# NVIDIA-RTX/RTXPT

Measured on AMD Instinct MI355X. Metric: Mrays/s at 4K 4spp 8-bounce bistro-like (extend + shadow rays / wall time of pt_render), higher is better.
Workload: dtype f32; 1 GPU; C3 bistro-like street canyon, 2808008 triangles, 64 materials, 32 textures 1024^2, 7368 emissive-triangle + env-quad lights, 3840x2160, 4 spp, 8 bounces, NEE 5 candidates + RR, lp types binary16 (reference default), environment cube 2048 BC6H (reference default on D3D12); BVH builder=PLOC + parallel re-insertion + cost-driven wide nodes, built on device, buildMs 79.1 (host part 0.0), 275780 wide n; parallelism=pixel-tile shard x1 + 1 gather, gather=none (1 GPU), transport=none, rehearsal=False

## Files before the change

rtxpt_amd/csrc/pt_api.hip:

```cpp
#include <cstring>
#include <rocprim/rocprim.hpp>
#include "pt_context.h"
#ifdef MI355PT_TEST_HOOKS
#include "../../include/mi355pt_testhooks.h"
#endif
#include "pt_denoiser.h"
#include <dlfcn.h>
#include <algorithm>
#include <cmath>
#include <cstdio>
#include <chrono>

using namespace ptk;

static_assert(sizeof(::PTMaterialData) == sizeof(ptk::PTMaterialData), "material ABI");
static_assert(sizeof(::PathTracerCameraData) == sizeof(ptk::PathTracerCameraData), "camera ABI");
static_assert(sizeof(::PtSettings) == sizeof(ptk::PtSettings), "settings ABI");
static_assert(sizeof(::PtGeometryDesc) == sizeof(ptk::GeometryDesc), "geometry ABI");
static_assert(sizeof(::PtInstanceDesc) == sizeof(ptk::InstanceDesc), "instance ABI");
static_assert(sizeof(::PolymorphicLightInfo) == sizeof(ptk::PolymorphicLightInfo), "light ABI");

namespace {

void build_mips(HostTexture& t) {
// ... 357 lines not shown
}
int bake_env_cube(pt_context* c) {
    ptk::EnvCube& e = c->envCube; memset(&e, 0, sizeof(e)); e.dim = c->envCubeDim; e.mipLevels = ptk::env_cube_mip_levels(e.dim);
    size_t total = 0; for (uint l = 0; l < e.mipLevels; l++) { e.mipOffset[l] = (uint)total; total += 6ull * (e.dim >> l) * (e.dim >> l); }
    PT_CHECK_HIP(c, c->dEnvCube.resize(total));
    std::vector<ptk::EnvDirectionalLight> dirLights = c->envDirLights;
    if (!c->sceneDirLights.empty()) {
        PtEnvMapSceneParams prm; memset(&prm, 0, sizeof(prm)); memcpy(prm.Transform, c->envToWorld.m, 48); prm.Enabled = 1.f;
        std::vector<ptk::EnvDirectionalLight> conv(c->sceneDirLights.size());
        if (pt_env_bake_lights(reinterpret_cast<const PtEnvDirectionalLight*>(c->sceneDirLights.data()), (uint32_t)conv.size(), &prm, e.dim, reinterpret_cast<PtEnvDirectionalLight*>(conv.data())) != PT_OK) return fail(c, PT_ERROR_INVALID_ARGUMENT, "scene directional lights");
        for (auto& l : conv) if (dirLights.size() < 16u) dirLights.push_back(l);
    }
    PT_CHECK_HIP(c, c->dEnvDirLights.upload(dirLights, c->stream));
    if (c->skyEnabled) {
        ptk::ProceduralSkyContext h = c->sky; h.Transmittance.texels = c->dSkyTex[0].p; h.Scatter.texels = c->dSkyTex[1].p; h.Irradiance.texels = c->dSkyTex[2].p; h.Clouds.texels = c->dSkyTex[3].p;
        PT_CHECK_HIP(c, c->dSky.resize(1)); PT_CHECK_HIP(c, hipMemcpyAsync(c->dSky.p, &h, sizeof(h), hipMemcpyHostToDevice, c->stream)); PT_CHECK_HIP(c, hipStreamSynchronize(c->stream));
        PT_CHECK_HIP(c, c->dSkyLowRes.resize(6ull * (e.dim / 2u) * (e.dim / 2u)));
    }
    refresh_scene_view(c);
    launch_env_cube_bake(c->dsc, c->dEnvDirLights.p, (uint)dirLights.size(), c->dEnvCube.p, c->dsc.envCube, c->stream);
    if (c->envCompression) {
        PT_CHECK_HIP(c, c->dEnvCubeSource.resize(total));
        PT_CHECK_HIP(c, hipMemcpyAsync(c->dEnvCubeSource.p, c->dEnvCube.p, sizeof(ptk::uint2) * total, hipMemcpyDeviceToDevice, c->stream));
        launch_env_cube_compress(c->dEnvCube.p, c->dsc.envCube, c->envCompression, c->stream);
    } else c->dEnvCubeSource.free();
    refresh_scene_view(c);
    PT_CHECK_HIP(c, hipGetLastError());
    c->envCubeDirty = false; c->lightsDirty = true;
    return PT_OK;
}
}

int prepare(pt_context* c) {
    if (c->texDirty) { int r = upload_textures(c); if (r != PT_OK) return r; refresh_scene_view(c); c->lightsDirty = true; c->envCubeDirty = true; }
    if (c->envEnabled && c->envCubeDirty) { int r = bake_env_cube(c); if (r != PT_OK) return r; }
    if (c->geomDirty) { int r = finalize_geometry(c); if (r != PT_OK) return r; }
    if (c->lightsDirty) { int r = bake_lights(c); if (r != PT_OK) return r; }
    else if (c->weightsDirty && !c->lights.empty()) {
        launch_light_weights(c->dLights.p, c->dLightsEx.p, (uint)c->lights.size(), c->dLightW.p, c->lightBoost, c->stream);
        int r = build_light_proxies(c, c->dLightW.p, nullptr, 0u, 0.f); if (r != PT_OK) return r;
        refresh_scene_view(c);
    }
    c->weightsDirty = false;
    return PT_OK;
}

int neeat_exchange_feedback(pt_context* c) {
    pt_context::NeeAt& st = c->neeat;
    if (c->shardCount == 1 || !c->comm || !st.feedbackFilled || st.W != c->width || st.H != c->height) return PT_OK;
    hipStream_t s = c->stream;
    if (st.xW != c->width || st.xH != c->height) {
        std::vector<uint> others; for (uint r = 0; r < c->shardCount; r++) if (r != c->shardRank) others.insert(others.end(), c->shardPixels[r].begin(), c->shardPixels[r].end());
        PT_CHECK_HIP(c, st.xPixels.upload(others, s)); PT_CHECK_HIP(c, st.xRecv.resize(3 * others.size())); PT_CHECK_HIP(c, st.xSend.resize(3 * c->owned.size())); PT_CHECK_HIP(c, hipStreamSynchronize(s));
        st.xW = c->width; st.xH = c->height;
    }
    const size_t n = c->owned.size();
    launch_pack_feedback(st.fbW.p, st.fbC.p, st.depth.p, c->dOwned.p, (uint)n, c->width, st.xSend.p, s);
    PT_CHECK_NCCL(c, g_rccl.GroupStart());
    size_t off = 0; ncclResult_t bad = ncclSuccess;
    for (uint r = 0; r < c->shardCount && bad == ncclSuccess; r++) {
        if (r == c->shardRank) continue;
        const size_t m = c->shardPixels[r].size();
        if (n) bad = g_rccl.Send(st.xSend.p, 3 * n, ncclFloat, (int)r, c->comm, s);
        if (m && bad == ncclSuccess) bad = g_rccl.Recv(st.xRecv.p + 3 * off, 3 * m, ncclFloat, (int)r, c->comm, s);
        off += m;
    }
    ncclResult_t ge = g_rccl.GroupEnd();
    if (bad != ncclSuccess || ge != ncclSuccess) return fail(c, PT_ERROR_HIP, std::string("NEE-AT feedback exchange: ") + g_rccl.GetErrorString(bad != ncclSuccess ? bad : ge));
    launch_unpack_feedback(st.fbW.p, st.fbC.p, st.depth.p, st.xPixels.p, (uint)off, c->width, st.xRecv.p, s);
    return PT_OK;
}
int neeat_frame(pt_context* c, int phases, const float* depth, const ptk::uint2* motion) {
    pt_context::NeeAt& st = c->neeat;
    const uint N = (uint)c->lights.size();
    if (!N || !c->numProxies) {
        c->localResX = c->localResY = c->localJitterX = c->localJitterY = c->localMaxLight = 0; c->localRatio = 0.f; c->feedbackRequired = false; st.feedbackFilled = st.lastFeedbackAvailable = false; st.frameOpen = false;
        refresh_scene_view(c); return PT_OK;
    }
    NeeAtFrame F; memset(&F, 0, sizeof(F));
    F.W = c->width; F.H = c->height; F.BW = (F.W + 1) / 2; F.BH = (F.H + 1) / 2; F.tilesX = (F.W + 7) / 8 + 1; F.tilesY = (F.H + 7) / 8 + 1;
    const size_t px = (size_t)F.W * F.H, bpx = (size_t)F.BW * F.BH, tiles = (size_t)F.tilesX * F.tilesY;
    if (phases & NEEAT_BEGIN) {
        if (st.historicTotalLightCount && st.historicTotalLightCount != N) st.feedbackFilled = st.lastFeedbackAvailable = false;
        if (st.W != F.W || st.H != F.H) {
            st.W = F.W; st.H = F.H; st.feedbackFilled = false; st.lastFeedbackAvailable = false;
            PT_CHECK_HIP(c, st.fbW.resize(px)); PT_CHECK_HIP(c, st.fbC.resize(px)); PT_CHECK_HIP(c, st.scW.resize(px)); PT_CHECK_HIP(c, st.scC.resize(px)); PT_CHECK_HIP(c, st.snapW.resize(px)); PT_CHECK_HIP(c, st.snapC.resize(px));
            PT_CHECK_HIP(c, st.blW.resize(bpx)); PT_CHECK_HIP(c, st.blC.resize(bpx)); PT_CHECK_HIP(c, st.local.resize(tiles * RTXPT_LIGHTING_LOCAL_PROXY_COUNT));
            PT_CHECK_HIP(c, hipMemsetAsync(st.fbW.p, 0, 4 * px, c->stream)); PT_CHECK_HIP(c, hipMemsetAsync(st.fbC.p, 0xFF, 4 * px, c->stream));
            PT_CHECK_HIP(c, st.depth.resize(px)); PT_CHECK_HIP(c, st.histDepth.resize(px));
            PT_CHECK_HIP(c, hipMemsetAsync(st.depth.p, 0, 4 * px, c->stream)); PT_CHECK_HIP(c, hipMemsetAsync(st.histDepth.p, 0, 4 * px, c->stream));
        }
        st.prevJitter[0] = st.jitter[0]; st.prevJitter[1] = st.jitter[1];
        neeat_advance_jitter(st.updateCounter, st.jitterF, st.jitter);
        st.updateCounter++;
        st.frameLocalAvailable = st.lastFeedbackAvailable; st.frameFeedbackAvailable = st.feedbackFilled;
        st.framePrevLightCount = st.historicTotalLightCount; st.historicTotalLightCount = N;
        st.frameOpen = true;
    }
    if (!st.frameOpen || st.W != F.W || st.H != F.H) return fail(c, PT_ERROR_NOT_READY, "NEE-AT: UpdateEnd without UpdateBegin of this frame size");
    const bool lastFrameLocalSamplesAvailable = st.frameLocalAvailable, lastFrameFeedbackAvailable = st.frameFeedbackAvailable;
    F.jitterX = st.jitter[0]; F.jitterY = st.jitter[1]; F.jitterPrevX = st.prevJitter[0]; F.jitterPrevY = st.prevJitter[1];
    F.updateCounter = st.updateCounter; F.dropoff = st.dropoff; F.totalLightCount = N; F.historicTotalLightCount = st.framePrevLightCount;
    F.lastFrameFeedbackAvailable = lastFrameFeedbackAvailable ? 1u : 0u; F.lastFrameLocalSamplesAvailable = (lastFrameLocalSamplesAvailable && lastFrameFeedbackAvailable) ? 1u : 0u;
    F.fbW = st.fbW.p; F.fbC = st.fbC.p; F.scW = st.scW.p; F.scC = st.scC.p; F.blW = st.blW.p; F.blC = st.blC.p; F.local = st.local.p;
    F.depth = depth ? depth : st.depth.p; F.motion = motion; F.historyDepth = st.histDepth.p; F.depthDisocclusionThreshold = 1.5f;
    const uint totalMaxFeedbackCount = lastFrameFeedbackAvailable ? ((F.W + 7) / 8) * ((F.H + 7) / 8) * 64u : 0u;
    if (phases & NEEAT_BEGIN) {
        PT_CHECK_HIP(c, st.counters.resize(N + 1)); PT_CHECK_HIP(c, hipMemsetAsync(st.counters.p, 0, 4 * (size_t)(N + 1), c->stream)); F.perLightCounters = st.counters.p;
        if (lastFrameFeedbackAvailable) launch_neeat_begin(F, st.snapW.p, st.snapC.p, st.preFilter, totalMaxFeedbackCount, c->stream);
        PT_CHECK_HIP(c, st.curW.resize(N + 1)); PT_CHECK_HIP(c, st.histW.resize(N));
        launch_neeat_boost_weights(c->dLightW.p, (lastFrameFeedbackAvailable && st.intensityDeltaMul > 0) ? st.histW.p : nullptr, st.nHist, N, st.intensityDeltaMul, st.curW.p, c->stream);
        int r = build_light_proxies(c, st.curW.p, lastFrameFeedbackAvailable ? st.counters.p : nullptr, totalMaxFeedbackCount, lastFrameFeedbackAvailable ? st.globalFeedbackWeight : 0.f); if (r != PT_OK) return r;
        PT_CHECK_HIP(c, hipMemcpyAsync(st.histW.p, st.curW.p, 4 * (size_t)N, hipMemcpyDeviceToDevice, c->stream)); st.nHist = N;
        st.lastFeedbackAvailable = lastFrameFeedbackAvailable;
    }
    if (!(phases & NEEAT_END)) { PT_CHECK_HIP(c, hipStreamSynchronize(c->stream)); return PT_OK; }
    F.perLightCounters = st.counters.p;
    F.samplingProxyCount = c->numProxies; F.proxies = c->dProxyIndices.p;
    launch_neeat_end(F, c->stream);
    if (!depth) PT_CHECK_HIP(c, hipMemsetAsync(st.depth.p, 0, 4 * px, c->stream));
    st.exportDepth = depth == nullptr;
    st.feedbackFilled = true; st.frameOpen = false;
    c->localResX = F.tilesX; c->localResY = F.tilesY; c->localJitterX = st.jitter[0]; c->localJitterY = st.jitter[1]; c->localMaxLight = 0;
    c->localRatio = lastFrameFeedbackAvailable ? st.localRatio : 0.f; c->sscThreshold = st.sscThreshold; c->feedbackRequired = true;
    refresh_scene_view(c);
    PT_CHECK_HIP(c, hipStreamSynchronize(c->stream));
    return PT_OK;
}

extern "C" {

int32_t pt_create(const PtDeviceDesc* desc, pt_context** out) {
    if (!out) return PT_ERROR_INVALID_ARGUMENT;
    *out = nullptr;
    int ndev = 0;
    if (hipGetDeviceCount(&ndev) != hipSuccess || ndev <= 0) return PT_ERROR_NO_DEVICE;
    int dev = desc ? desc->deviceOrdinal : 0;
    if (dev < 0 || dev >= ndev) return PT_ERROR_INVALID_ARGUMENT;
    if (hipSetDevice(dev) != hipSuccess) return PT_ERROR_HIP;
    pt_context* c = new pt_context();
    c->device = dev; c->shardRank = desc ? desc->shardRank : 0; c->shardCount = (desc && desc->shardCount) ? desc->shardCount : 1;
    if (c->shardRank >= c->shardCount) { delete c; return PT_ERROR_INVALID_ARGUMENT; }
    if (hipStreamCreateWithFlags(&c->stream, hipStreamNonBlocking) != hipSuccess) { delete c; return PT_ERROR_HIP; }
    c->streams[0] = c->stream;
    for (uint b = 1; b < PT_PIPELINE_BATCHES; b++) if (hipStreamCreateWithFlags(&c->streams[b], hipStreamNonBlocking) != hipSuccess) { delete c; return PT_ERROR_HIP; }
    if (hipHostMalloc(&c->hostCounters, PT_PIPELINE_BATCHES * sizeof(WaveCounters), hipHostMallocDefault) != hipSuccess) { delete c; return PT_ERROR_HIP; }
    c->serialKernels = desc && (desc->flags & PT_DEVICE_SERIAL_KERNELS);
    c->bvhBuilder = (desc && (desc->flags & PT_DEVICE_PREFER_FAST_BUILD)) ? BVH_BUILDER_PLOC : ((desc && (desc->flags & PT_DEVICE_HOST_SAH_BUILDER)) ? BVH_BUILDER_SAH : BVH_BUILDER_PLOC_OPT);
    { const char* e = getenv("MI355PT_BVH_BUILDER");
      if (e && !strcmp(e, "karras")) c->bvhBuilder = BVH_BUILDER_KARRAS; else if (e && !strcmp(e, "ploc")) c->bvhBuilder = BVH_BUILDER_PLOC; else if (e && !strcmp(e, "sah")) c->bvhBuilder = BVH_BUILDER_SAH; else if (e && (!strcmp(e, "ploc_opt") || !strcmp(e, "device"))) c->bvhBuilder = BVH_BUILDER_PLOC_OPT; }
    { const char* e = getenv("MI355PT_TAIL_PATHS"); if (e) c->tailBelow = (uint)strtoul(e, nullptr, 10); }
    { const char* e = getenv("MI355PT_COMPACT_POOL"); if (e) c->compactPool = atoi(e) != 0; }
    { const char* e = getenv("MI355PT_FIRST_VERTEX_IN_PLACE"); if (e) c->firstVertexInPlace = atoi(e) != 0; }
    { const char* e = getenv("MI355PT_FUSED_TRAVERSAL"); if (e) c->fusedTraversal = (uint)strtoul(e, nullptr, 10); }
    { const char* e = getenv("MI355PT_DROP_INERT_TERMINAL"); if (e) c->dropInertTerminal = atoi(e) != 0; }
    { const char* e = getenv("MI355PT_TAIL_DEFER"); if (e) c->tailDefer = (uint)strtoul(e, nullptr, 10); }
    memset(&c->dsc, 0, sizeof(c->dsc)); memset(&c->cam, 0, sizeof(c->cam)); memset(&c->bvh, 0, sizeof(c->bvh));
    pt_default_settings(reinterpret_cast<::PtSettings*>(&c->S));
    const float I[12] = {1, 0, 0, 0, 0, 1, 0, 0, 0, 0, 1, 0}; memcpy(c->envToWorld.m, I, 48); memcpy(c->envToLocal.m, I, 48); c->envColorMul = ptk::make_float3(1.0f / ptk::kEnvMapRadianceScale);
    if (c->dCounters.resize(PT_PIPELINE_BATCHES) != hipSuccess) { delete c; return PT_ERROR_HIP; }
    *out = c;
    return PT_OK;
}
int32_t pt_destroy(pt_context* c) {
    if (!c) return PT_ERROR_INVALID_ARGUMENT;
    (void)hipSetDevice(c->device); (void)hipStreamSynchronize(c->stream);
    if (c->comm && g_rccl.lib) { (void)g_rccl.CommDestroy(c->comm); c->comm = nullptr; }
    c->dSpHeader.free(); c->dSpThroughput.free(); c->dSpPlanes.free(); c->dSpRadiance.free(); c->dSpMotion.free(); c->dSpDepth.free(); c->dSpHitT.free(); c->dSpMark.free(); c->dSpNewL.free(); c->dSpScratch.free(); c->dSpGatherSend.free(); c->dSpGatherRecv.free(); c->dSpGatherPixels.free();
    c->dDnRRDiff.free(); c->dDnRRSpec.free(); c->dDnRRSpecMV.free(); c->dDnRRNormal.free(); c->dDnMotion.free(); c->dDnViewZ.free(); c->dDnRoughness.free(); c->dDnNormal.free(); c->dDnDiff.free(); c->dDnSpec.free(); c->dDnDisocclusion.free(); c->dDnHistoryClamp.free();
    relax_free(c); taa_free(c); bloom_free(c); taau_free(c);
    c->neeat.free(); c->dLocalTable.free(); c->dFbWeight.free(); c->dFbCand.free(); c->dSq3.free();
    c->dGatherSend.free(); c->dGatherRecv.free(); c->dGatherPixels.free(); c->dLightW.free(); c->dProxyOffsets.free(); if (c->dScanTemp) (void)hipFree(c->dScanTemp);
    if (c->bvhAllocated) bvh_free(c->bvh);
    c->dIndices.free(); c->dNormals.free(); c->dTangents.free(); c->dProxyCounters.free(); c->dProxyIndices.free(); c->dEnvLookup.free(); c->dOwned.free(); c->dQueue[0].free(); c->dQueue[1].free();
    c->dPrevPositions.free(); c->dPrevInstances.free(); c->dEmissiveList.free(); c->dEmissiveOffsets.free(); c->dPositions.free(); c->dUvs.free(); c->dGeometries.free(); c->dInstances.free(); c->dSubInstances.free(); c->dSubInstToInstGeom.free();
    c->dPrimInfo.free(); c->dShadeTris.free(); c->dInertBits.free(); c->dAlphaPlanes.free(); c->dAlphaPool.free(); c->dMaterials.free(); c->dTexInfos.free(); c->dTexels.free(); c->dEnvCube.free(); c->dEnvCubeSource.free(); c->dEnvImageCube.free(); c->dEnvDirLights.free(); c->dLights.free(); c->dLightsEx.free(); c->dS0.free(); c->dS1.free(); c->dS2.free(); c->dS3.free(); c->dS4.free();
    c->dHit.free(); c->dS0b.free(); c->dS1b.free(); c->dS3b.free(); c->dS4b.free(); c->dHitb.free(); c->dSq0.free(); c->dSq1.free(); c->dSq2.free(); c->dAccum.free(); c->dScratch4.free(); c->dCounters.free(); c->dTravSpill.free(); c->dTaskQ.free(); c->dTravCounts.free(); c->dResolveList.free(); c->dBestKey.free(); c->dResolveListSh.free(); c->dBestKeySh.free(); c->dTaskQSh.free();
    for (uint b = 1; b < PT_PIPELINE_BATCHES; b++) (void)hipStreamDestroy(c->streams[b]);
    (void)hipStreamDestroy(c->stream); (void)hipHostFree(c->hostCounters);
    delete c;
    return PT_OK;
}
const char* pt_get_last_error(pt_context* c) { return c ? c->lastError.c_str() : "null context"; }

int32_t pt_set_geometry(pt_context* c, const PtGeometryBuffers* b, const PtGeometryDesc* geoms, uint32_t nGeoms, const PtMeshDesc* meshes, uint32_t nMeshes) {
    if (!c || !b || !geoms || !meshes) return fail(c, PT_ERROR_INVALID_ARGUMENT, "null argument");
    if (!b->indices || !b->positions) return fail(c, PT_ERROR_INVALID_ARGUMENT, "indices and positions are required");
    for (uint32_t g = 0; g < nGeoms; g++) {
        if ((size_t)geoms[g].indexOffset + geoms[g].numIndices > b->numIndices || (size_t)geoms[g].vertexOffset + geoms[g].numVertices > b->numVertices || geoms[g].numIndices % 3)
            return fail(c, PT_ERROR_INVALID_ARGUMENT, "geometry range outside the supplied streams");
        if ((geoms[g].flags & PT_GEOM_HAS_UV) && !b->uvs) return fail(c, PT_ERROR_INVALID_ARGUMENT, "geometry has uv flag but no uv stream");
        if ((geoms[g].flags & PT_GEOM_HAS_NORMAL) && !b->normals) return fail(c, PT_ERROR_INVALID_ARGUMENT, "geometry has normal flag but no normal stream");
        if ((geoms[g].flags & PT_GEOM_HAS_TANGENT) && !b->tangents) return fail(c, PT_ERROR_INVALID_ARGUMENT, "geometry has tangent flag but no tangent stream");
        const uint32_t* idx = b->indices + geoms[g].indexOffset;
        for (uint32_t k = 0; k < geoms[g].numIndices; k++) if (idx[k] >= geoms[g].numVertices) return fail(c, PT_ERROR_INVALID_ARGUMENT, "index outside the geometry's vertex range");
    }
    for (uint32_t m = 0; m < nMeshes; m++)
        if ((size_t)meshes[m].firstGeometry + meshes[m].numGeometries > nGeoms) return fail(c, PT_ERROR_INVALID_ARGUMENT, "mesh references geometries outside the supplied array");
    uint nv = b->numVertices;
    c->indices.assign(b->indices, b->indices + b->numIndices);
    c->positions.assign(b->positions, b->positions + 3 * (size_t)nv);
    c->uvs.assign(nv, ptk::make_float2(0, 0)); if (b->uvs) memcpy(c->uvs.data(), b->uvs, 8 * (size_t)nv);
    c->normals.assign(nv, 0); if (b->normals) memcpy(c->normals.data(), b->normals, 4 * (size_t)nv);
    c->tangents.assign(nv, 0); if (b->tangents) memcpy(c->tangents.data(), b->tangents, 4 * (size_t)nv);
    c->geometries.resize(nGeoms); memcpy(c->geometries.data(), geoms, sizeof(GeometryDesc) * nGeoms);
    c->meshes.resize(nMeshes); memcpy(c->meshes.data(), meshes, sizeof(MeshDesc) * nMeshes);
    c->geomDirty = true;
    relax_drop_history(c); taa_drop_history(c); taau_drop_history(c);
    return PT_OK;
}
int32_t pt_set_instances(pt_context* c, const PtInstanceDesc* inst, uint32_t n) {
    if (!c || (!inst && n)) return fail(c, PT_ERROR_INVALID_ARGUMENT, "null argument");
    c->instances.resize(n); if (n) memcpy(c->instances.data(), inst, sizeof(InstanceDesc) * n);
    c->geomDirty = true;
    return PT_OK;
}
int32_t pt_set_materials(pt_context* c, const ::PTMaterialData* mats, uint32_t nMats, const PtTextureDesc* tex, uint32_t nTex) {
    if (!c || (!mats && nMats) || (!tex && nTex)) return fail(c, PT_ERROR_INVALID_ARGUMENT, "null argument");
    c->materials.resize(nMats); if (nMats) memcpy(c->materials.data(), mats, 128 * (size_t)nMats);
    c->textures.clear();
    for (uint32_t i = 0; i < nTex; i++) {
        const PtTextureDesc& d = tex[i];
        if (!d.pixels || !d.width || !d.height || d.format > 2) return fail(c, PT_ERROR_INVALID_ARGUMENT, "bad texture descriptor");
        if (d.width > 32768u || d.height > 32768u) return fail(c, PT_ERROR_UNSUPPORTED, "textures above 32768 texels per side are not supported (16 mip levels)");
        HostTexture t; t.w = d.width; t.h = d.height; t.mips.resize(1); t.mips[0].resize((size_t)d.width * d.height);
        for (size_t k = 0; k < (size_t)d.width * d.height; k++) {
            ptk::float4 v;
            if (d.format == PT_TEX_RGBA32F) { const float* p = (const float*)d.pixels + 4 * k; v = ptk::make_float4(p[0], p[1], p[2], p[3]); }
            else {
                const uint8_t* p = (const uint8_t*)d.pixels + 4 * k;
                v = ptk::make_float4((float)p[0] / 255.0f, (float)p[1] / 255.0f, (float)p[2] / 255.0f, (float)p[3] / 255.0f);
                if (d.format == PT_TEX_RGBA8_SRGB) { v.x = srgb_to_linear(v.x); v.y = srgb_to_linear(v.y); v.z = srgb_to_linear(v.z); }
            }
            t.mips[0][k] = v;
        }
        build_mips(t);
        c->textures.push_back(std::move(t));
    }
    for (uint32_t m = 0; m < nMats; m++) {
        const ptk::PTMaterialData& mm = c->materials[m];
        auto chk = [&](uint flag, uint word) { return !(mm.Flags & flag) || (word & 0xFFFFu) < nTex; };
        if (!chk(PTMaterialFlags_UseBaseOrDiffuseTexture, mm.BaseOrDiffuseTextureIndex) || !chk(PTMaterialFlags_UseEmissiveTexture, mm.EmissiveTextureIndex) ||
            !chk(PTMaterialFlags_UseNormalTexture, mm.NormalTextureIndex) || !chk(PTMaterialFlags_UseMetalRoughOrSpecularTexture, mm.MetalRoughOrSpecularTextureIndex) ||
            !chk(PTMaterialFlags_UseTransmissionTexture, mm.TransmissionTextureIndex))
            return fail(c, PT_ERROR_INVALID_ARGUMENT, "material references a missing texture");
    }
    c->texDirty = true; c->geomDirty = true;
    return PT_OK;
}
static void set_env_params(pt_context* c, const PtEnvMapSceneParams* params) {
    if (params) {
        memcpy(c->envToWorld.m, params->Transform, 48);
        memset(&c->envToLocal, 0, sizeof(float3x4));
        for (int r = 0; r < 3; r++) for (int k = 0; k < 3; k++) c->envToLocal.m[r * 4 + k] = c->envToWorld.m[k * 4 + r];
        c->envColorMul = ptk::make_float3(params->ColorMultiplier[0], params->ColorMultiplier[1], params->ColorMultiplier[2]);
    } else {
        const float I[12] = {1, 0, 0, 0, 0, 1, 0, 0, 0, 0, 1, 0}; memcpy(c->envToWorld.m, I, 48); memcpy(c->envToLocal.m, I, 48);
        c->envColorMul = ptk::make_float3(1.0f / ptk::kEnvMapRadianceScale);
    }
}
static bool env_has_image(const pt_context* c) { return c->envTex.w != 0u || c->envImageCubeDim != 0u; }
int32_t pt_set_environment(pt_context* c, const float* rgb, uint32_t w, uint32_t h, const PtEnvMapSceneParams* params) {
    if (!c) return PT_ERROR_INVALID_ARGUMENT;
    c->envImageCubeDim = 0; c->dEnvImageCube.free();
    c->envEnabled = (w != 0 && h != 0 && rgb && (!params || params->Enabled != 0.f));
    if (!c->envEnabled) { c->envTex.w = c->envTex.h = 0; c->envTex.mips.clear(); if (c->skyEnabled && (!params || params->Enabled != 0.f)) c->envEnabled = true; }
    else {
        HostTexture& t = c->envTex; t.w = w; t.h = h; t.mips.clear(); t.mips.resize(1); t.mips[0].resize((size_t)w * h);
        for (size_t i = 0; i < (size_t)w * h; i++) t.mips[0][i] = ptk::make_float4(rgb[3 * i], rgb[3 * i + 1], rgb[3 * i + 2], 1.f);
        t.mipLevels = 1;
    }
    set_env_params(c, params);
    c->texDirty = true; c->lightsDirty = true; c->envCubeDirty = true;
    return PT_OK;
}
int32_t pt_set_environment_cube(pt_context* c, const float* rgbaFaces, uint32_t dim, const PtEnvMapSceneParams* params) {
    if (!c) return PT_ERROR_INVALID_ARGUMENT;
    if (dim > 16384u) return fail(c, PT_ERROR_INVALID_ARGUMENT, "cube-map source: at most 16384 texels per side");
    c->envTex.w = c->envTex.h = 0; c->envTex.mips.clear();
    c->envEnabled = (dim != 0 && rgbaFaces && (!params || params->Enabled != 0.f));
    if (!c->envEnabled) { c->envImageCubeDim = 0; c->dEnvImageCube.free(); if (c->skyEnabled && (!params || params->Enabled != 0.f)) c->envEnabled = true; }
    else {
        const size_t n = 6ull * dim * dim; std::vector<ptk::uint2> h(n);
        for (size_t i = 0; i < n; i++) h[i] = ptk::env_pack_rgba16f(ptk::make_float4(rgbaFaces[4 * i], rgbaFaces[4 * i + 1], rgbaFaces[4 * i + 2], rgbaFaces[4 * i + 3]));
        PT_CHECK_HIP(c, c->dEnvImageCube.resize(n)); PT_CHECK_HIP(c, hipMemcpy(c->dEnvImageCube.p, h.data(), n * sizeof(ptk::uint2), hipMemcpyHostToDevice));
        c->envImageCubeDim = dim;
    }
    set_env_params(c, params);
    c->texDirty = true; c->lightsDirty = true; c->envCubeDirty = true;
    return PT_OK;
}
int32_t pt_set_procedural_sky(pt_context* c, const PtProceduralSkyConstants* consts, const PtProceduralSkyTextures* tex) {
    if (!c) return PT_ERROR_INVALID_ARGUMENT;
    static_assert(sizeof(PtProceduralSkyConstants) == sizeof(ptk::ProceduralSkyConstants), "ProceduralSkyConstants layout");
    if (!consts) {
        if (c->skyEnabled) { c->skyEnabled = false; if (!env_has_image(c)) c->envEnabled = false; c->envCubeDirty = true; c->lightsDirty = true; c->texDirty = true; }
        return PT_OK;
    }
    if (tex) {
        const PtSkyTexture* t[4] = {&tex->transmittance, &tex->scattering, &tex->irradiance, &tex->clouds}; ptk::SkyTexture* dst[4] = {&c->sky.Transmittance, &c->sky.Scatter, &c->sky.Irradiance, &c->sky.Clouds};
        for (int i = 0; i < 4; i++) {
            if (!t[i]->rgba || !t[i]->width || !t[i]->height || !t[i]->depth || t[i]->width > 4096u || t[i]->height > 4096u || t[i]->depth > 4096u) return fail(c, PT_ERROR_INVALID_ARGUMENT, "procedural sky: every look-up texture needs RGBA float texels and sizes in [1, 4096]");
            if ((i == 0 || i == 2) && t[i]->depth != 1u) return fail(c, PT_ERROR_INVALID_ARGUMENT, "procedural sky: the transmittance and irradiance textures are 2-D (depth 1)");
        }
        for (int i = 0; i < 4; i++) {
            const size_t n = (size_t)t[i]->width * t[i]->height * t[i]->depth;
            PT_CHECK_HIP(c, c->dSkyTex[i].resize(n)); PT_CHECK_HIP(c, hipMemcpy(c->dSkyTex[i].p, t[i]->rgba, n * sizeof(ptk::float4), hipMemcpyHostToDevice));
            dst[i]->texels = nullptr; dst[i]->w = t[i]->width; dst[i]->h = t[i]->height; dst[i]->d = t[i]->depth; dst[i]->_pad = 0u;
        }
    } else if (!c->dSkyTex[0].p) return fail(c, PT_ERROR_INVALID_ARGUMENT, "procedural sky: no look-up textures have been set yet");
    memcpy(&c->sky.Consts, consts, sizeof(ptk::ProceduralSkyConstants));
    if (!c->envEnabled) {
        if (!env_has_image(c)) { const float I[12] = {1, 0, 0, 0, 0, 1, 0, 0, 0, 0, 1, 0}; memcpy(c->envToWorld.m, I, 48); memcpy(c->envToLocal.m, I, 48); c->envColorMul = ptk::make_float3(1.0f / ptk::kEnvMapRadianceScale); }
        c->envEnabled = true; c->texDirty = true;
    }
    c->skyEnabled = true; c->envCubeDirty = true; c->lightsDirty = true;
    return PT_OK;
}
int32_t pt_set_environment_bake(pt_context* c, uint32_t cubeDim, const PtEnvDirectionalLight* lights, uint32_t n) {
    if (!c || (!lights && n)) return fail(c, PT_ERROR_INVALID_ARGUMENT, "null argument");
    if (cubeDim && (cubeDim < 16u || cubeDim > 8192u || (cubeDim & (cubeDim - 1u)))) return fail(c, PT_ERROR_INVALID_ARGUMENT, "cube resolution must be a power of two in [16, 8192]");
    if (n > 16u) return fail(c, PT_ERROR_INVALID_ARGUMENT, "at most 16 directional lights are baked into the environment cube (EnvMapBaker.hlsl: EMB_MAXDIRLIGHTS)");
    if (cubeDim) c->envCubeDim = cubeDim;
    static_assert(sizeof(PtEnvDirectionalLight) == sizeof(ptk::EnvDirectionalLight), "EnvDirectionalLight layout");
    c->envDirLights.resize(n); if (n) memcpy(c->envDirLights.data(), lights, sizeof(ptk::EnvDirectionalLight) * n);
    c->envCubeDirty = true; c->lightsDirty = true;
    return PT_OK;
}
int32_t pt_set_scene_directional_lights(pt_context* c, const PtEnvDirectionalLight* worldLights, uint32_t n) {
    if (!c || (!worldLights && n)) return fail(c, PT_ERROR_INVALID_ARGUMENT, "null argument");
// ... 914 lines not shown
```

rtxpt_amd/csrc/pt_context.h:

```cpp
#pragma once
#include "../../include/mi355pt.h"
#include "pt_wavefront.h"
#include "pt_stableplanes_launch.h"
#include "pt_denoiser.h"
#include "pt_build.h"
#include <rccl/rccl.h>
#include <string>
#include <vector>

#pragma GCC visibility push(hidden)

using namespace ptk;

template <typename T> struct DevBuf {
    T* p = nullptr; size_t n = 0;
    hipError_t resize(size_t count) {
        if (count <= n && p) return hipSuccess;
        if (p) (void)hipFree(p);
        p = nullptr; n = 0;
        hipError_t e = hipMalloc(&p, sizeof(T) * (count ? count : 1));
        if (e == hipSuccess) n = count ? count : 1;
        return e;
    }
    hipError_t upload(const T* src, size_t count, hipStream_t st) {
        hipError_t e = resize(count); if (e != hipSuccess) return e;
        if (!count) return hipSuccess;
        return hipMemcpyAsync(p, src, sizeof(T) * count, hipMemcpyHostToDevice, st);
    }
    hipError_t upload(const std::vector<T>& v, hipStream_t st) { return upload(v.data(), v.size(), st); }
    void free() { if (p) (void)hipFree(p); p = nullptr; n = 0; }
};

struct HostTexture { uint w, h, mipLevels; std::vector<std::vector<ptk::float4>> mips; };

static const uint TILE = 32;
static const uint TASK_QUEUE_CAPACITY = 1u << 22;
#ifndef PT_SHARD_TILE_GROUP
#define PT_SHARD_TILE_GROUP 1
#endif
#ifndef PT_PIPELINE_FULL_AT
#define PT_PIPELINE_FULL_AT (1u << 21)
#endif
#ifndef PT_PIPELINE_MID_BATCHES
#define PT_PIPELINE_MID_BATCHES 2
#endif
#ifndef PT_CLASSIFY_FROM
#define PT_CLASSIFY_FROM 65536u
#endif
#ifndef PT_SP_FILL_CLASSES
#define PT_SP_FILL_CLASSES 1
#endif
#ifndef PT_SP_FILL_RANGED
#define PT_SP_FILL_RANGED 1
#endif
#ifndef PT_TAIL_PATHS
#define PT_TAIL_PATHS 4096u
#endif
#ifndef PT_FUSED_TRAVERSAL
#define PT_FUSED_TRAVERSAL 1u
#endif
#ifndef PT_FUSED_BELOW
#define PT_FUSED_BELOW (12u << 20)
#endif
#ifndef PT_COMPACT_POOL
#define PT_COMPACT_POOL 1
#endif
#ifndef PT_FIRST_VERTEX_IN_PLACE
#define PT_FIRST_VERTEX_IN_PLACE 1
#endif
#ifndef PT_DROP_INERT_TERMINAL
#define PT_DROP_INERT_TERMINAL 1
#endif
#ifndef PT_FREE_RUN_BELOW
#define PT_FREE_RUN_BELOW (1u << 22)
#endif
#ifndef PT_PIPELINE_BATCHES
#define PT_PIPELINE_BATCHES 4
#endif

#pragma GCC visibility pop
struct pt_context {
    int device = 0; hipStream_t stream = nullptr; uint shardRank = 0, shardCount = 1;
    hipStream_t streams[PT_PIPELINE_BATCHES] = {}; WaveCounters* hostCounters = nullptr; bool serialKernels = false;
    uint tailBelow = PT_TAIL_PATHS, tailDefer = 0, fusedTraversal = PT_FUSED_TRAVERSAL; bool compactPool = PT_COMPACT_POOL != 0, firstVertexInPlace = PT_FIRST_VERTEX_IN_PLACE != 0;
    bool dropInertTerminal = PT_DROP_INERT_TERMINAL != 0; unsigned long long droppedTerminal = 0;
    std::string lastError;
    std::vector<uint> indices; std::vector<float> positions; std::vector<ptk::float2> uvs; std::vector<uint> normals, tangents;
    std::vector<GeometryDesc> geometries; std::vector<MeshDesc> meshes; std::vector<InstanceDesc> instances;
    std::vector<ptk::PTMaterialData> materials; std::vector<HostTexture> textures; HostTexture envTex; bool envEnabled = false;
    float3x4 envToWorld, envToLocal; ptk::float3 envColorMul;
    uint envCubeDim = 2048; std::vector<ptk::EnvDirectionalLight> envDirLights, sceneDirLights; bool envCubeDirty = true;
    ptk::EnvCube envCube;
    std::vector<PolymorphicLightInfoFull> analyticLights;
    std::vector<SubInstanceData> subInstances; std::vector<ptk::uint2> subInstToInstGeom; std::vector<ptk::uint2> primInfo;
    std::vector<uint> subInstFirstPrim;
    std::vector<ptk::PolymorphicLightInfo> lights; std::vector<ptk::PolymorphicLightInfoEx> lightsEx; std::vector<uint> envLookup;
    uint envLookupDim = 0; uint numProxies = 0, envLightsBaked = 0;
    DevBuf<float> dLightW; DevBuf<uint> dProxyOffsets; void* dScanTemp = nullptr; size_t scanTempBytes = 0;
    DevBuf<uint> dIndices, dNormals, dTangents, dProxyCounters, dProxyIndices, dEnvLookup, dOwned, dQueue[2], dEmissiveList, dEmissiveOffsets;
    DevBuf<float> dPrevPositions; DevBuf<InstanceDesc> dPrevInstances; bool motionHistory = false, prevAllStale = false;
    std::vector<uint32_t> prevStaleRanges;
    DevBuf<float> dPositions; DevBuf<ptk::float2> dUvs; DevBuf<GeometryDesc> dGeometries; DevBuf<InstanceDesc> dInstances;
    DevBuf<SubInstanceData> dSubInstances;
    DevBuf<ptk::AlphaPlane> dAlphaPlanes; DevBuf<unsigned char> dAlphaPool; DevBuf<ptk::ShadeTri> dShadeTris;
    DevBuf<uint> dInertBits;
    DevBuf<ptk::uint2> dSubInstToInstGeom, dPrimInfo; DevBuf<ptk::PTMaterialData> dMaterials; DevBuf<TexInfo> dTexInfos; DevBuf<ptk::float4> dTexels;
    bool skyEnabled = false; ptk::ProceduralSkyContext sky; DevBuf<ptk::float4> dSkyTex[4]; DevBuf<ptk::ProceduralSkyContext> dSky;
    DevBuf<ptk::uint2> dSkyLowRes;
    DevBuf<ptk::uint2> dEnvImageCube; uint envImageCubeDim = 0;
    DevBuf<ptk::uint2> dEnvCube, dEnvCubeSource; DevBuf<ptk::EnvDirectionalLight> dEnvDirLights; uint envCompression = 0;
    DevBuf<ptk::PolymorphicLightInfo> dLights; DevBuf<ptk::PolymorphicLightInfoEx> dLightsEx;
    DevBuf<uint> dLocalTable; uint localResX = 0, localResY = 0, localJitterX = 0, localJitterY = 0, localMaxLight = 0;
    float localRatio = 0.f, sscThreshold = 0.f; bool feedbackRequired = false;
    DevBuf<float> dFbWeight; DevBuf<uint> dFbCand; DevBuf<ptk::float4> dSq3; uint fbSamples = 0;
    ptk::LightFrustumBoost lightBoost = {}; bool weightsDirty = false;
    struct NeeAt {
        bool enabled = false; float globalFeedbackWeight = 0.75f, localRatio = 0.65f, sscThreshold = 0.3f, dropoff = 0.005f, intensityDeltaMul = 64.0f;
        bool preFilter = true;
        uint updateCounter = 0; float jitterF[2] = {0, 0}; uint jitter[2] = {0, 0}, prevJitter[2] = {0, 0};
        bool feedbackFilled = false, lastFeedbackAvailable = false; uint historicTotalLightCount = 0, W = 0, H = 0, nHist = 0;
        bool frameOpen = false, frameFeedbackAvailable = false, frameLocalAvailable = false, exportDepth = true; uint framePrevLightCount = 0;
        DevBuf<float> fbW, scW, blW, snapW, curW, histW; DevBuf<uint> fbC, scC, blC, snapC, local, counters;
        DevBuf<float> depth, histDepth; bool haveClip = false; float clipZ[4] = {0, 0, 0, 0}, clipW[4] = {0, 0, 0, 0};
        DevBuf<uint> xSend, xRecv; DevBuf<uint> xPixels; uint xW = 0, xH = 0;
        void reset() {
            W = H = 0; updateCounter = 0; jitterF[0] = jitterF[1] = 0; jitter[0] = jitter[1] = prevJitter[0] = prevJitter[1] = 0;
            feedbackFilled = lastFeedbackAvailable = false; frameOpen = false; exportDepth = true; historicTotalLightCount = 0; nHist = 0;
        }
        void free() {
            fbW.free(); scW.free(); blW.free(); snapW.free(); curW.free(); histW.free(); fbC.free(); scC.free(); blC.free(); snapC.free();
            local.free(); counters.free(); xSend.free(); xRecv.free(); xPixels.free(); depth.free(); histDepth.free();
        }
    } neeat;
    DevBuf<ptk::uint4> dS0, dS1, dS2, dS3, dS4, dHit, dS0b, dS1b, dS3b, dS4b, dHitb; DevBuf<ptk::float4> dSq0, dSq1, dSq2, dAccum, dScratch4;
    DevBuf<WaveCounters> dCounters; DevBuf<ptk::uint2> dTravSpill; DevBuf<ptk::TravTask> dTaskQ; DevBuf<uint> dTravCounts, dResolveList;
    DevBuf<unsigned long long> dBestKey;
    DevBuf<ptk::TravTask> dTaskQSh; DevBuf<uint> dResolveListSh; DevBuf<unsigned long long> dBestKeySh;
    std::vector<TexInfo> texInfos; TexInfo envTexInfo;
    BvhBuildBuffers bvh; bool bvhAllocated = false; uint numTris = 0; uint bvhBuilder = BVH_BUILDER_SAH;
    DeviceScene dsc;
    ptk::PtSettings S; ptk::PathTracerCameraData cam; uint width = 0, height = 0, accumCount = 0; std::vector<uint> owned;
    std::vector<std::vector<uint>> shardPixels;
    std::vector<float> hostRadiance; bool countersEnabled = false;
    bool geomDirty = true, lightsDirty = true, texDirty = true;
    double buildMs = 0, refitMs = 0, lightBakeMs = 0;
    uint poolCapacity = 0; size_t shadowCapacity = 0;
    DevBuf<uint> dSpHeader, dSpThroughput; DevBuf<ptk::StablePlane> dSpPlanes; DevBuf<ptk::uint2> dSpRadiance, dSpMotion;
    DevBuf<float> dSpDepth, dSpHitT; uint spW = 0, spH = 0; bool spGathered = false;
    DevBuf<ptk::uint4> dSpMark; DevBuf<ptk::float4> dSpNewL;
    DevBuf<float> dSpScratch; DevBuf<uint> dSpGatherSend, dSpGatherRecv, dSpGatherPixels; uint spGatherW = 0, spGatherH = 0;
    DevBuf<uint> dDnRRDiff, dDnRRSpec, dDnRRSpecMV; DevBuf<ptk::uint2> dDnRRNormal, dDnMotion; DevBuf<float> dDnViewZ, dDnRoughness;
    DevBuf<ptk::float4> dDnNormal, dDnDiff, dDnSpec;
    DevBuf<unsigned char> dDnDisocclusion, dDnHistoryClamp; uint dnW = 0, dnH = 0;
    uint spSampleBase = 0;
    DevBuf<ptk::float4> dRxHist[3][2][5], dRxOut[3][2], dRxGuide, dRxPing[2], dRxPong[2];
    uint rxW = 0, rxH = 0, rxSide[3] = {0, 0, 0}; bool rxHistory[3] = {false, false, false}, rxDenoised[3] = {false, false, false}; int dnPreparedPlane = -1;
    uint spFrameSerial = 0, rxFrameSerial[3] = {0, 0, 0};
    bool rxTiming = false; std::vector<float> rxPassMs; std::vector<hipEvent_t> rxEvents;
    DevBuf<ptk::float4> dTaa[2]; uint taaW = 0, taaH = 0, taaSide = 0, taaFrameSerial = 0, dnNrdSerial = 0; bool taaHistory = false, taaResolved = false;
    hipEvent_t taaEvents[2] = {nullptr, nullptr};
    DevBuf<ptk::float4> dBloom, dBloomQ[2]; uint bloomW = 0, bloomH = 0; bool bloomReady = false;
    hipEvent_t bloomEvents[2] = {nullptr, nullptr};
    DevBuf<ptk::float4> dTaau[2], dTaauBloom, dTaauBloomQ[2]; uint taauW = 0, taauH = 0, taauRenderW = 0, taauRenderH = 0, taauSide = 0, taauFrameSerial = 0;
    bool taauHistory = false, taauResolved = false, taauBloomReady = false;
    hipEvent_t taauEvents[2] = {nullptr, nullptr}, taauBloomEvents[2] = {nullptr, nullptr};
    ncclComm_t comm = nullptr; uint commRank = 0, commWorld = 0; DevBuf<ptk::float4> dGatherSend, dGatherRecv; DevBuf<uint> dGatherPixels;
    std::vector<size_t> gatherCounts; uint gatherW = 0, gatherH = 0;
};

#pragma GCC visibility push(hidden)

inline int fail(pt_context* c, int code, const std::string& msg) { if (c) c->lastError = msg; return code; }
#define PT_CHECK_HIP(c, expr) \
    do { hipError_t e_ = (expr); if (e_ != hipSuccess) return fail(c, PT_ERROR_HIP, std::string(#expr) + ": " + hipGetErrorString(e_)); } while (0)

int prepare(pt_context* c);
int neeat_exchange_feedback(pt_context* c);
enum { NEEAT_BEGIN = 1, NEEAT_END = 2, NEEAT_BOTH = 3 };
int neeat_frame(pt_context* c, int phases = NEEAT_BOTH, const float* depth = nullptr, const ptk::uint2* motion = nullptr);
inline int32_t dn_ready(pt_context* c) {
    if (!c->spW || c->spW != c->width || c->spH != c->height) return fail(c, PT_ERROR_NOT_READY, "no stable planes of this frame size yet: pt_build_stable_planes, pt_fill_stable_planes");
    if (c->shardCount > 1 && !c->spGathered) return fail(c, PT_ERROR_NOT_READY, "the denoiser passes read the whole frame's planes: pt_gather_stable_planes / pt_unpack_stable_planes first");
    return PT_OK;
}
inline ptk::DenoiserBuffers dn_buffers(pt_context* c) {
    ptk::DenoiserBuffers D;
    D.RRDiffuseAlbedo = c->dDnRRDiff.p; D.RRSpecAlbedo = c->dDnRRSpec.p; D.RRNormalsAndRoughness = c->dDnRRNormal.p; D.RRSpecMotionVectors = c->dDnRRSpecMV.p;
    D.ViewZ = c->dDnViewZ.p; D.MotionVectors = c->dDnMotion.p; D.NormalRoughness = c->dDnNormal.p; D.DiffRadianceHitDist = c->dDnDiff.p; D.SpecRadianceHitDist = c->dDnSpec.p;
    D.Roughness = c->dDnRoughness.p; D.DisocclusionThresholdMix = c->dDnDisocclusion.p; D.CombinedHistoryClampRelax = c->dDnHistoryClamp.p;
    return D;
}
void relax_drop_history(pt_context* c);
void relax_free(pt_context* c);
void taa_drop_history(pt_context* c);
void taa_free(pt_context* c);
int32_t taa_resolved_ready(pt_context* c);
void bloom_drop(pt_context* c);
void bloom_free(pt_context* c);
void taau_drop_history(pt_context* c);
void taau_free(pt_context* c);
StablePlanesContext sp_context(pt_context* c, const PtStablePlanesParams* params);
void add_frame_stats(PtFrameStats& t, const PtFrameStats& o);

#pragma GCC visibility pop
```

rtxpt_amd/csrc/pt_frame.hip:

```cpp
#include "pt_context.h"
#include <cstdio>
#include <cstdlib>
#include <cstring>

StablePlanesContext sp_context(pt_context* c, const PtStablePlanesParams* params) {
    ptk::StablePlanesParams prm;
    if (params) memcpy(&prm, params, sizeof(prm));
    else { memset(&prm, 0, sizeof(prm)); prm.activeStablePlaneCount = cStablePlaneCount; }
    StablePlanesContext sp; sp.C = ptk::SP_make_consts(prm, c->width, c->height, c->S.bounceCount);
    sp.B.Header = c->dSpHeader.p; sp.B.Planes = c->dSpPlanes.p; sp.B.StableRadiance = c->dSpRadiance.p; sp.B.Depth = c->dSpDepth.p;
    sp.B.SpecularHitT = c->dSpHitT.p; sp.B.MotionVectors = c->dSpMotion.p; sp.B.Throughput = c->dSpThroughput.p;
    return sp;
}

void add_frame_stats(PtFrameStats& t, const PtFrameStats& o) {
    t.extendRays += o.extendRays; t.shadowRays += o.shadowRays; t.hits += o.hits;
    t.nodeVisitsExtend += o.nodeVisitsExtend; t.triTestsExtend += o.triTestsExtend; t.nodeVisitsShadow += o.nodeVisitsShadow;
    t.triTestsShadow += o.triTestsShadow; t.leafVisitsExtend += o.leafVisitsExtend; t.waveItersExtend += o.waveItersExtend;
    t.leafVisitsShadow += o.leafVisitsShadow; t.waveItersShadow += o.waveItersShadow;
    for (int q = 0; q < 4; q++) t.extendPhaseCycles[q] += o.extendPhaseCycles[q];
    t.leafBlocksExtend += o.leafBlocksExtend; if (o.waveItersMaxExtend > t.waveItersMaxExtend) t.waveItersMaxExtend = o.waveItersMaxExtend;
    for (int q = 0; q < 16; q++) t.extendRayIterHist[q] += o.extendRayIterHist[q];
    for (uint q = 0; q < o.longRayCount && q < 32u && t.longRayCount < 32u; q++) { memcpy(t.longRays[t.longRayCount], o.longRays[q], 32); t.longRayCount++; }
    for (int q = 0; q < 8; q++) t.extendEvents[q] += o.extendEvents[q];
    t.gpuMilliseconds += o.gpuMilliseconds; t.extendKernelMs += o.extendKernelMs; t.shadeKernelMs += o.shadeKernelMs; t.shadowKernelMs += o.shadowKernelMs;
    t.extendLaunches += o.extendLaunches; if (o.iterations > t.iterations) t.iterations = o.iterations;
    t.pathsTraced += o.pathsTraced; t.tailLaunches += o.tailLaunches;
}

namespace {


int ensure_pool(pt_context* c, uint n, uint shadowPerPath) {
    if (n <= c->poolCapacity && (size_t)n * shadowPerPath <= c->shadowCapacity) return PT_OK;
    if (n < c->poolCapacity) n = c->poolCapacity;
    const size_t ns = (size_t)n * shadowPerPath;
    if (ns > 0xF0000000ull) return fail(c, PT_ERROR_INVALID_ARGUMENT, "too many shadow-queue entries in one pt_render call (paths x NEEFullSamples)");
    PT_CHECK_HIP(c, c->dS0.resize(n)); PT_CHECK_HIP(c, c->dS1.resize(n)); PT_CHECK_HIP(c, c->dS2.resize(n)); PT_CHECK_HIP(c, c->dS3.resize(n));
    PT_CHECK_HIP(c, c->dS4.resize(n)); PT_CHECK_HIP(c, c->dHit.resize(n)); PT_CHECK_HIP(c, c->dQueue[0].resize(n)); PT_CHECK_HIP(c, c->dQueue[1].resize(n));
    PT_CHECK_HIP(c, c->dSq0.resize(ns)); PT_CHECK_HIP(c, c->dSq1.resize(ns)); PT_CHECK_HIP(c, c->dSq2.resize(ns));
    PT_CHECK_HIP(c, c->dBestKey.resize(ns)); PT_CHECK_HIP(c, c->dResolveList.resize(ns));
    PT_CHECK_HIP(c, c->dTaskQ.resize((size_t)PT_PIPELINE_BATCHES * 2 * TASK_QUEUE_CAPACITY));
    PT_CHECK_HIP(c, c->dTravCounts.resize(PT_PIPELINE_BATCHES * PASS_COUNTERS));
    c->poolCapacity = n; c->shadowCapacity = ns;
    return PT_OK;
}

struct Events {
    std::vector<hipEvent_t> ev;
    Events() = default; Events(const Events&) = delete; Events& operator=(const Events&) = delete;
    ~Events() { for (hipEvent_t e : ev) if (e) (void)hipEventDestroy(e); }
    hipError_t record(hipStream_t st) {
        hipEvent_t e = nullptr; const hipError_t r = hipEventCreate(&e); ev.push_back(e);
        return r != hipSuccess ? r : hipEventRecord(e, st);
    }
    size_t mark(hipStream_t st) { (void)record(st); return ev.size() - 1; }
    float ms(size_t a = 0, size_t b = 1) const { float m = 0; (void)hipEventElapsedTime(&m, ev[a], ev[b]); return m; }
};

struct Batch {
    uint pixFirst = 0, numPix = 0, total = 0, base = 0;
    hipStream_t st = nullptr; WaveCounters* wc = nullptr; WaveCounters* hwc = nullptr;
    PathPool pool; ShadowQueue sq; uint* queue[2] = {nullptr, nullptr}; DeviceScene sc; PathKernelContext k; TravAux aux;
    uint cur = 0, active = 0, iterations = 0; unsigned long long extendRays = 0, shadowRays = 0; bool waiting = false;
};
uint batch_count(const pt_context* c, uint paths) {
    if (c->serialKernels || paths < (1u << 20)) return 1u;
    return paths < PT_PIPELINE_FULL_AT ? (uint)PT_PIPELINE_MID_BATCHES : (uint)PT_PIPELINE_BATCHES;
}
void slice_batch(pt_context* c, const PathKernelContext& k, uint b, uint numBatches, uint pathsPerPixel, uint shadowPerPath,
                 const ShadowQueue& frameSq, uint maxBlocks, Batch& t) {
    const unsigned long long numOwned = c->owned.size();
    t.pixFirst = (uint)(numOwned * b / numBatches); t.numPix = (uint)(numOwned * (b + 1) / numBatches) - t.pixFirst;
    t.total = t.numPix * pathsPerPixel; t.base = t.pixFirst * pathsPerPixel;
    t.st = c->streams[b]; t.wc = c->dCounters.p + b; t.hwc = c->hostCounters + b;
    t.pool = PathPool{c->dS0.p + t.base, c->dS1.p + t.base, c->dS2.p + t.base, c->dS3.p + t.base, c->dS4.p + t.base, c->dHit.p + t.base};
    const size_t sbase = (size_t)t.base * shadowPerPath;
    t.sq = frameSq; t.sq.q0 += sbase; t.sq.q1 += sbase; t.sq.q2 += sbase; if (t.sq.q3) t.sq.q3 += sbase;
    t.queue[0] = c->dQueue[0].p + t.base; t.queue[1] = c->dQueue[1].p + t.base;
    t.sc = c->dsc; t.sc.travSpill = c->dsc.travSpill + (size_t)b * T8_MAX_BLOCKS * T8_GROUPS_PER_BLOCK * T8_SPILL_DEPTH;
    t.k = k; t.k.sc = t.sc;
    t.aux.taskQ[0] = c->dTaskQ.p + (size_t)(2 * b) * TASK_QUEUE_CAPACITY; t.aux.taskQ[1] = t.aux.taskQ[0] + TASK_QUEUE_CAPACITY;
    t.aux.counts = c->dTravCounts.p + PASS_COUNTERS * b; t.aux.taskCap = TASK_QUEUE_CAPACITY; t.aux.maxBlocks = maxBlocks;
    t.aux.bestKey = c->dBestKey.p + sbase; t.aux.resolveList = c->dResolveList.p + sbase; t.aux.primToSlot = c->bvh.primToSlot;
    memset(t.hwc, 0, sizeof(WaveCounters));
}
PathKernelContext kernel_context(const pt_context* c) { PathKernelContext k; k.sc = c->dsc; k.S = c->S; k.cam = c->cam; return k; }
ShadowQueue frame_shadow_queue(const pt_context* c, uint group) {
    return ShadowQueue{c->dSq0.p, c->dSq1.p, c->dSq2.p, group, nullptr, nullptr, nullptr, 0u, 0u, 0u};
}
TravAux shadow_aux(const Batch& t) { TravAux a = t.aux; a.counts = t.aux.counts + PASS_SHADOW_OFFSET; return a; }

uint nested_dielectric_allowance(const ptk::PtSettings& S) { return S.nestedDielectricsQuality == 2 ? 16u : (S.nestedDielectricsQuality == 1 ? 4u : 0u); }

bool composed_frame(const pt_context* c, uint shadowGroup) { return !c->serialKernels && !c->countersEnabled && !shadowGroup && c->dsc.rootIsValid; }

PtFrameStats batch_stats(const Batch& t, uint shadowGroup) {
    const WaveCounters& h = *t.hwc;
    PtFrameStats s; memset(&s, 0, sizeof(s));
    s.extendRays = t.extendRays + h.tailExtendRays; s.shadowRays = shadowGroup ? h.shadowValid : t.shadowRays + h.tailShadowRays; s.hits = h.hits;
    s.nodeVisitsExtend = h.nodeVisitsExt; s.triTestsExtend = h.triTestsExt; s.nodeVisitsShadow = h.nodeVisitsSh; s.triTestsShadow = h.triTestsSh;
    s.leafVisitsExtend = h.leafVisitsExt; s.waveItersExtend = h.itersExt; s.leafVisitsShadow = h.leafVisitsSh; s.waveItersShadow = h.itersSh;
    for (int q = 0; q < 4; q++) s.extendPhaseCycles[q] = h.phaseCycExt[q];
    s.leafBlocksExtend = h.leafBlocksExt; s.waveItersMaxExtend = h.itersMaxExt;
    for (int q = 0; q < 8; q++) s.extendEvents[q] = h.eventsExt[q];
    for (int q = 0; q < 16; q++) s.extendRayIterHist[q] = h.rayIterHistExt[q];
    s.longRayCount = h.longRayCount < 32u ? h.longRayCount : 32u; memcpy(s.longRays, h.longRays, 32 * (size_t)s.longRayCount);
    s.extendLaunches = s.iterations = t.iterations; s.pathsTraced = t.total;
    return s;
}

template <typename B> int32_t check_frame_end(pt_context* c, const B* batches, uint numBatches, const char* stillAlive) {
    for (uint b = 0; b < numBatches; b++)
        if (batches[b].hwc->overflow)
            return fail(c, PT_ERROR_HIP, "BVH8 traversal: stack tail or straggler task queue overflow (raise T8_SPILL_DEPTH / TASK_QUEUE_CAPACITY)");
    for (uint b = 0; b < numBatches; b++) if (batches[b].active) return fail(c, PT_ERROR_HIP, stillAlive);
    return PT_OK;
}
template <typename B> int32_t drain_frame(pt_context* c, B* batches, uint numBatches, Events& frame) {
    for (uint b = 0; b < numBatches; b++)
        PT_CHECK_HIP(c, hipMemcpyAsync(batches[b].hwc, batches[b].wc, sizeof(WaveCounters), hipMemcpyDeviceToHost, batches[b].st));
    for (uint b = 0; b < numBatches; b++) PT_CHECK_HIP(c, hipStreamSynchronize(batches[b].st));
    PT_CHECK_HIP(c, frame.record(c->stream));
    PT_CHECK_HIP(c, hipStreamSynchronize(c->stream));
    PT_CHECK_HIP(c, hipGetLastError());
    return PT_OK;
}


struct RenderBatch : Batch {
    uint bound = 0;
    uint tailLaunches = 0; bool afterTail = false, inTail = false;
    uint pendingShadow = 0; TravAux auxSh;
    PathPool poolSet[2]; uint set = 0; bool compact = false;
    bool firstInPlace = false;
    bool timed = false; Events marks; size_t t0 = 0, t1 = 0;
    struct Span { size_t a, b; int kind; uint items; }; std::vector<Span> spans;
    size_t mark() { return timed ? marks.mark(st) : 0; }
    void span(size_t a, size_t b, int kind, uint items) { if (timed) spans.push_back({a, b, kind, items}); }
};

struct RenderFrame {
    pt_context* c; uint first, count, total, shadowGroup, shadowPerPath; bool feedback;
    uint numBatches = 0; RenderBatch B[PT_PIPELINE_BATCHES];
    uint maxIter = 0, tailBelow = 0, wavefrontPasses = 0; bool fused = false, passLog = false;

    bool live(const RenderBatch& t) const { return t.active && t.bound < maxIter; }
    int32_t setup(const PathKernelContext& k) {
        numBatches = batch_count(c, total);
        static const uint batchesOverride = []() { const char* e = getenv("MI355PT_BATCHES"); return e ? (uint)strtoul(e, nullptr, 10) : 0u; }();
        static const uint blocksOverride = []() { const char* e = getenv("MI355PT_MAX_BLOCKS"); return e ? (uint)strtoul(e, nullptr, 10) : 0u; }();
        if (batchesOverride && !c->serialKernels) numBatches = batchesOverride < (uint)PT_PIPELINE_BATCHES ? batchesOverride : (uint)PT_PIPELINE_BATCHES;
        uint maxBlocks = (numBatches >= 3u) ? (total < (6u << 20) ? 256u * 7u / 2u : (total < (24u << 20) ? 256u * 35u / 8u : 256u * 7u)) : 0u;
        if (blocksOverride) maxBlocks = blocksOverride < 2u ? 2u : (blocksOverride < T8_MAX_BLOCKS ? blocksOverride : (uint)T8_MAX_BLOCKS);
        ShadowQueue sq = frame_shadow_queue(c, shadowGroup);
        if (feedback) {
            sq.q3 = c->dSq3.p; sq.fbTotalWeight = c->neeat.enabled ? c->neeat.fbW.p : c->dFbWeight.p;
            sq.fbCandidates = c->neeat.enabled ? c->neeat.fbC.p : c->dFbCand.p;
            sq.fbWidth = c->width; sq.fbPlane = c->width * c->height; sq.fbSampleFirst = first;
        }
        passLog = getenv("MI355PT_PASS_LOG") != nullptr;
        for (uint b = 0; b < numBatches; b++) {
            RenderBatch& t = B[b];
            slice_batch(c, k, b, numBatches, count, shadowPerPath, sq, maxBlocks, t);
            t.timed = c->serialKernels || c->countersEnabled || passLog;
            t.hwc->extendCount[0] = t.active = t.total;
        }
        maxIter = c->S.bounceCount + 2 + nested_dielectric_allowance(c->S);
        const bool composed = composed_frame(c, shadowGroup);
        tailBelow = composed ? c->tailBelow : 0u;
        const bool fuse = composed && (c->fusedTraversal == 1u || (c->fusedTraversal == 2u && total < PT_FUSED_BELOW));
        if (fuse) { int32_t r = enable_fused(); if (r != PT_OK) return r; }
        const bool neeatShade = c->dsc.lights.LocalSamplingBuffer != nullptr || c->dsc.lights.TemporalFeedbackRequired != 0u;
        if (composed && c->compactPool && !neeatShade && !feedback) {
            int32_t r = enable_compact_pool(); if (r != PT_OK) return r;
            if (c->firstVertexInPlace) enable_first_vertex_in_place();
        }
        return PT_OK;
    }
    int32_t enable_fused() {
        PT_CHECK_HIP(c, c->dBestKeySh.resize(c->shadowCapacity)); PT_CHECK_HIP(c, c->dResolveListSh.resize(c->shadowCapacity));
        PT_CHECK_HIP(c, c->dTaskQSh.resize((size_t)PT_PIPELINE_BATCHES * 2 * TASK_QUEUE_CAPACITY));
        for (uint b = 0; b < numBatches; b++) {
            RenderBatch& t = B[b]; const size_t sbase = (size_t)t.base * shadowPerPath;
            t.auxSh = shadow_aux(t);
            t.auxSh.taskQ[0] = c->dTaskQSh.p + (size_t)(2 * b) * TASK_QUEUE_CAPACITY; t.auxSh.taskQ[1] = t.auxSh.taskQ[0] + TASK_QUEUE_CAPACITY;
            t.auxSh.bestKey = c->dBestKeySh.p + sbase; t.auxSh.resolveList = c->dResolveListSh.p + sbase;
        }
        fused = true;
        return PT_OK;
    }
    int32_t enable_compact_pool() {
        PT_CHECK_HIP(c, c->dS0b.resize(c->poolCapacity)); PT_CHECK_HIP(c, c->dS1b.resize(c->poolCapacity)); PT_CHECK_HIP(c, c->dS3b.resize(c->poolCapacity));
        PT_CHECK_HIP(c, c->dS4b.resize(c->poolCapacity)); PT_CHECK_HIP(c, c->dHitb.resize(c->poolCapacity));
        for (uint b = 0; b < numBatches; b++) {
            RenderBatch& t = B[b]; t.compact = true; t.set = 0; t.poolSet[0] = t.pool;
            t.poolSet[1] = PathPool{c->dS0b.p + t.base, c->dS1b.p + t.base, t.pool.s2, c->dS3b.p + t.base, c->dS4b.p + t.base, c->dHitb.p + t.base, nullptr};
        }
        return PT_OK;
    }
    void enable_first_vertex_in_place() {
        for (uint b = 0; b < numBatches; b++) {
            RenderBatch& t = B[b]; t.firstInPlace = t.compact && !(tailBelow && t.total <= tailBelow);
            t.hwc->firstCamera.cam = t.k.cam; t.hwc->firstCamera.perPixelJitterAAScale = t.k.S.perPixelJitterAAScale;
        }
    }
    int32_t start() {
        for (uint b = 0; b < numBatches; b++) {
            RenderBatch& t = B[b];
            t.t0 = t.mark();
            PT_CHECK_HIP(c, hipMemcpyAsync(t.wc, t.hwc, sizeof(WaveCounters), hipMemcpyHostToDevice, t.st));
            if (!t.firstInPlace) launch_generate(t.k, t.pool, c->dOwned.p + t.pixFirst, t.numPix, first, count, 0u, t.total, t.queue[0], nullptr, t.st);
        }
        return PT_OK;
    }
    int32_t queue_pass(RenderBatch& t) {
        const uint nxt = t.cur ^ 1u;
        launch_pass_reset(t.aux.counts, &t.wc->extendCount[nxt], fused ? nullptr : &t.wc->shadowCount, t.st);
        if (tailBelow && t.active <= tailBelow && !t.afterTail) return queue_tail(t);
        t.afterTail = false; t.bound++; wavefrontPasses++;
        const size_t e0 = t.mark();
        PathPool pin = t.pool, pout = PathPool{};
        if (t.compact) { pin = t.poolSet[t.set]; pin.home = t.queue[t.cur]; pout = t.poolSet[t.set ^ 1u]; t.set ^= 1u; }
        const uint* countIn = &t.wc->extendCount[t.cur];
        const bool vertex0 = t.firstInPlace && t.iterations == 0u;
        const FirstVertex fv{c->dOwned.p + t.pixFirst, t.numPix, first, count};
        if (vertex0) launch_extend_first(t.k, pin, fv, countIn, t.active, t.wc, t.aux, t.st);
        else if (t.pendingShadow) {
            launch_trace_pair(t.sc, pin, t.queue[t.cur], countIn, t.active, t.sq, &t.wc->shadowCount, t.pendingShadow, t.wc, t.aux, t.auxSh, t.st);
            t.pendingShadow = 0;
        } else launch_extend(t.sc, pin, t.queue[t.cur], countIn, t.active, t.wc, c->countersEnabled, t.aux, t.st);
        const size_t e1 = t.mark(); t.span(e0, e1, 0, t.active);
        uint* classScratch = t.active >= PT_CLASSIFY_FROM ? reinterpret_cast<uint*>(t.aux.bestKey) : nullptr;
        launch_shade(t.k, pin, t.queue[t.cur], countIn, t.active, t.queue[nxt], &t.wc->extendCount[nxt], t.sq, t.wc, classScratch,
                     t.aux.counts + PASS_CLASS_OFFSET, t.st, pout, vertex0 ? &fv : nullptr, c->dropInertTerminal ? c->dInertBits.p : nullptr);
        const size_t e2 = t.mark(); t.span(e1, e2, 1, t.active);
        t.extendRays += t.active;
        PT_CHECK_HIP(c, hipMemcpyAsync(t.hwc, t.wc, 16, hipMemcpyDeviceToHost, t.st));
        t.waiting = true;
        return PT_OK;
    }
    int32_t queue_tail(RenderBatch& t) {
        const uint nxt = t.cur ^ 1u;
        if (t.compact) {
            PathPool in = t.poolSet[t.set]; in.home = t.queue[t.cur];
            launch_uncompact(in, t.poolSet[t.set ^ 1u], &t.wc->extendCount[t.cur], t.active, t.st);
            t.pool = t.poolSet[t.set ^ 1u]; t.compact = false;
        }
        if (t.pendingShadow) {
            launch_shadow(t.sc, t.pool, t.sq, &t.wc->shadowCount, t.pendingShadow, t.wc, false, t.auxSh, t.st);
            PT_CHECK_HIP(c, hipMemsetAsync(&t.wc->shadowCount, 0, 4, t.st));
            t.pendingShadow = 0;
        }
        const size_t e0 = t.mark();
        launch_tail(t.k, t.pool, t.queue[t.cur], &t.wc->extendCount[t.cur], t.active, t.queue[nxt], &t.wc->extendCount[nxt], t.sq, t.wc, maxIter - t.bound,
                    c->tailDefer, t.aux.maxBlocks, t.st);
        const size_t e1 = t.mark(); t.span(e0, e1, 3, t.active);
        t.tailLaunches++; t.afterTail = true; t.inTail = true;
        PT_CHECK_HIP(c, hipMemcpyAsync(t.hwc, t.wc, 16, hipMemcpyDeviceToHost, t.st));
        t.waiting = true;
        return PT_OK;
    }
    int32_t finish_pass(RenderBatch& t, uint b) {
        t.waiting = false; t.inTail = false;
        const uint nxt = t.cur ^ 1u, nShadow = t.hwc->shadowCount;
        if (passLog) {
            uint pc[PASS_COUNTERS]; PT_CHECK_HIP(c, hipMemcpy(pc, t.aux.counts, sizeof(pc), hipMemcpyDeviceToHost));
            fprintf(stderr, "[pass log]   b%u pass %u: %u paths -> extend splits %u / %u / %u / %u sub-trees, %u rays resolved; %u visibility rays next\n",
                    b, t.iterations, t.active, pc[0], pc[1], pc[2], pc[3], pc[TRAV_RESOLVE], nShadow);
            if (t.active >= PT_CLASSIFY_FROM)
                fprintf(stderr, "[pass log]   b%u pass %u: classes %u continuing / %u terminating / %u misses, %u inert terminating hits dropped\n",
                        b, t.iterations, pc[PASS_CLASS_OFFSET], pc[PASS_CLASS_OFFSET + 1], pc[PASS_CLASS_OFFSET + 2], pc[PASS_CLASS_OFFSET + 3]);
        }
        t.active = t.hwc->extendCount[nxt];
        if (fused && nShadow && live(t)) { t.pendingShadow = nShadow; t.shadowRays += nShadow; }
        else if (nShadow) {
            const size_t s0 = t.mark();
            launch_shadow(t.sc, t.pool, t.sq, &t.wc->shadowCount, nShadow, t.wc, c->countersEnabled, fused ? t.auxSh : shadow_aux(t), t.st);
            const size_t s1 = t.mark(); t.span(s0, s1, 2, nShadow);
            if (!shadowGroup) t.shadowRays += nShadow;
            if (fused) PT_CHECK_HIP(c, hipMemsetAsync(&t.wc->shadowCount, 0, 4, t.st));
        }
        t.cur = nxt; t.iterations++;
        return PT_OK;
    }
    int32_t lockstep() {
        static const uint freeRunBelow = []() {
            const char* e = getenv("MI355PT_FREE_RUN_BELOW"); return e ? (uint)strtoul(e, nullptr, 10) : (uint)PT_FREE_RUN_BELOW;
        }();
        for (;;) {
            bool freeRun = freeRunBelow != 0u && numBatches > 1u;
            for (uint b = 0; b < numBatches; b++) if (live(B[b]) && B[b].active >= freeRunBelow) freeRun = false;
            wavefrontPasses = 0;
            for (uint b = 0; b < numBatches; b++) {
                RenderBatch& t = B[b];
                if (t.waiting || !live(t)) continue;
                int32_t r = queue_pass(t); if (r != PT_OK) return r;
            }
            if (freeRun) return PT_OK;
            bool any = false;
            for (uint b = 0; b < numBatches; b++) {
                RenderBatch& t = B[b];
                if (!t.waiting) continue;
                if (t.inTail && wavefrontPasses && hipStreamQuery(t.st) == hipErrorNotReady) { any = true; continue; }
                PT_CHECK_HIP(c, hipStreamSynchronize(t.st));
                int32_t r = finish_pass(t, b); if (r != PT_OK) return r;
                if (live(t)) any = true;
            }
            if (!any) return PT_OK;
        }
    }
    int32_t free_run() {
        uint waiting = 0; for (uint b = 0; b < numBatches; b++) waiting += B[b].waiting ? 1u : 0u;
        while (waiting) {
            for (uint b = 0; b < numBatches; b++) {
                RenderBatch& t = B[b];
                if (!t.waiting || hipStreamQuery(t.st) == hipErrorNotReady) continue;
                PT_CHECK_HIP(c, hipStreamSynchronize(t.st));
                int32_t r = finish_pass(t, b); if (r != PT_OK) return r;
                waiting--;
                if (live(t)) { r = queue_pass(t); if (r != PT_OK) return r; waiting++; }
            }
        }
        return PT_OK;
    }
    void accumulate() {
        for (uint b = 0; b < numBatches; b++) {
            RenderBatch& t = B[b];
            launch_accumulate(t.pool, c->dOwned.p + t.pixFirst, t.numPix, count, c->dAccum.p, c->accumCount, c->width, t.st);
            t.t1 = t.mark();
        }
    }
    void harvest(PtFrameStats& stats, float frameMs) const {
        for (uint b = 0; b < numBatches; b++) {
            const RenderBatch& t = B[b];
            PtFrameStats s = batch_stats(t, shadowGroup);
            s.tailLaunches = t.tailLaunches;
            for (const RenderBatch::Span& sp : t.spans) {
                const float m = t.marks.ms(sp.a, sp.b);
                if (sp.kind == 0) s.extendKernelMs += m; else if (sp.kind == 1) s.shadeKernelMs += m; else if (sp.kind == 2) s.shadowKernelMs += m;
            }
            add_frame_stats(stats, s);
        }
        stats.gpuMilliseconds = frameMs;
    }
    void log_passes() const {
        static const char* const kinds[4] = {"extend", "shade", "shadow", "tail"};
        for (uint b = 0; b < numBatches; b++) {
            const RenderBatch& t = B[b]; const WaveCounters& h = *t.hwc;
            if (t.tailLaunches)
                fprintf(stderr, "[pass log] batch %u: %u tail launches traced %llu + %llu rays, handed back %llu extend stragglers, "
                        "%llu visibility stragglers, %llu paths at the bounce bound\n", b, t.tailLaunches, (unsigned long long)h.tailExtendRays,
                        (unsigned long long)h.tailShadowRays, (unsigned long long)h.tailHandedBack[0], (unsigned long long)h.tailHandedBack[1],
                        (unsigned long long)h.tailHandedBack[2]);
            if (!t.timed) continue;
            fprintf(stderr, "[pass log] batch %u of %u: %u paths, %u passes, %.3f ms from first to last event\n", b, numBatches, t.total, t.iterations,
                    t.marks.ms(t.t0, t.t1));
            for (const RenderBatch::Span& sp : t.spans)
                fprintf(stderr, "[pass log]   b%u %-6s %9u items  start %8.3f ms  %7.3f ms\n", b, kinds[sp.kind], sp.items, t.marks.ms(t.t0, sp.a),
                        t.marks.ms(sp.a, sp.b));
        }
    }
};

int32_t render_sample_by_sample(pt_context* c, uint32_t first, uint32_t count, PtFrameStats* stats) {
    PtFrameStats total; memset(&total, 0, sizeof(total));
    int32_t r = PT_OK;
    for (uint32_t s = 0; s < count && r == PT_OK; s++) {
        PtFrameStats one; r = pt_render(c, first + s, 1, &one);
        if (r == PT_OK) add_frame_stats(total, one);
    }
    if (stats) *stats = total;
    return r;
}
int32_t prepare_neeat_layers(pt_context* c, uint32_t count, bool feedback, uint shadowGroup) {
    if (c->localResX) {
        const uint TILE_PX = ptk::RTXPT_LIGHTING_SAMPLING_BUFFER_TILE_SIZE;
        if ((c->width - 1u + c->localJitterX) / TILE_PX >= c->localResX || (c->height - 1u + c->localJitterY) / TILE_PX >= c->localResY)
            return fail(c, PT_ERROR_INVALID_ARGUMENT, "local sampling table smaller than the frame");
        if (c->localMaxLight >= c->lights.size())
            return fail(c, PT_ERROR_INVALID_ARGUMENT, "local sampling table names a light index beyond the baked light table");
    }
    c->fbSamples = 0;
    if (!feedback) return PT_OK;
    if (shadowGroup)
        return fail(c, PT_ERROR_INVALID_ARGUMENT, "NEE-AT temporal feedback needs NEEFullSamples 1 (the reference's default): the feedback draw of one light "
                                                  "sample shifts the random numbers of the next");
    const size_t plane = (size_t)c->width * c->height;
    PT_CHECK_HIP(c, c->dSq3.resize(c->shadowCapacity));
    if (!c->neeat.enabled) {
        PT_CHECK_HIP(c, c->dFbWeight.resize(plane * count)); PT_CHECK_HIP(c, c->dFbCand.resize(plane * count));
        PT_CHECK_HIP(c, hipMemsetAsync(c->dFbWeight.p, 0, 4 * plane * count, c->stream));
        PT_CHECK_HIP(c, hipMemsetAsync(c->dFbCand.p, 0xFF, 4 * plane * count, c->stream));
    }
    PT_CHECK_HIP(c, hipStreamSynchronize(c->stream));
    return PT_OK;
}


struct FillBatch : Batch { PathPool markPool; ptk::float4* newL = nullptr; };

struct FillFrame {
    pt_context* c; StablePlanesContext sp; uint sampleIndex; bool feedback;
    uint numBatches = 0, maxIter = 0; FillBatch B[PT_PIPELINE_BATCHES];

    bool live(const FillBatch& t) const { return t.active && t.iterations < maxIter; }
    void commit() { for (uint b = 0; b < numBatches; b++) launch_sp_fill_commit(B[b].k, sp, B[b].pool, B[b].numPix, sampleIndex, B[b].st); }
    void setup(const PathKernelContext& k) {
        numBatches = batch_count(c, (uint)c->owned.size());
        ShadowQueue sq = frame_shadow_queue(c, 0u);
        if (feedback) {
            sq.q3 = c->dSq3.p; sq.fbTotalWeight = c->neeat.fbW.p; sq.fbCandidates = c->neeat.fbC.p;
            sq.fbWidth = c->width; sq.fbPlane = 0u; sq.fbSampleFirst = 0u;
        }
        for (uint b = 0; b < numBatches; b++) {
            FillBatch& t = B[b];
            slice_batch(c, k, b, numBatches, 1u, 1u, sq, (numBatches >= 3u) ? 256u * 7u : 0u, t);
            t.markPool = t.pool; t.markPool.s2 = c->dSpMark.p + t.base; t.newL = c->dSpNewL.p + t.base;
        }
        maxIter = c->S.bounceCount + 2 + nested_dielectric_allowance(c->S) * (c->S.bounceCount + 1u);
    }
    int32_t start() {
// ... 196 lines not shown
```

rtxpt_amd/csrc/pt_wavefront.h:

```cpp
#pragma once
#include "pt_path.h"
#include "pt_neeat.h"
#include "pt_tonemap.h"
#include <hip/hip_runtime.h>

namespace ptk {

struct PathPool { uint4* s0; uint4* s1; uint4* s2; uint4* s3; uint4* s4; uint4* hit;
    const uint* home; };
struct ShadowQueue { float4* q0; float4* q1; float4* q2; uint group;
    float4* q3; float* fbTotalWeight; uint* fbCandidates; uint fbWidth, fbPlane, fbSampleFirst; };
struct FirstVertex { const uint* ownedPixels; uint numOwned, sampleFirst, spp; };
struct FirstVertexCamera { PathTracerCameraData cam; float perPixelJitterAAScale, _pad[3]; };
struct WaveCounters {
    uint extendCount[2]; uint shadowCount; uint overflow;
    unsigned long long hits, nodeVisitsExt, triTestsExt, nodeVisitsSh, triTestsSh, leafVisitsExt, itersExt, leafVisitsSh, itersSh, phaseCycExt[4], leafBlocksExt, eventsExt[8], itersMaxExt, rayIterHistExt[16]; uint longRayCount, _padLong; float longRays[32][8];
    unsigned long long shadowValid;
    unsigned long long tailExtendRays, tailShadowRays;
    unsigned long long tailHandedBack[3];
    unsigned long long droppedTerminal;
    FirstVertexCamera firstCamera;
};

static const uint TRAV_COUNTERS = 5, TRAV_RESOLVE = 4, PASS_COUNTERS = 16, PASS_SHADOW_OFFSET = 5, PASS_CLASS_OFFSET = 10;
struct TravAux { TravTask* taskQ[2]; uint* counts; uint taskCap; unsigned long long* bestKey; uint* resolveList; const uint* primToSlot; uint maxBlocks; };

void launch_generate(const PathKernelContext& k, PathPool pool, const uint* ownedPixels, uint numOwned, uint sampleFirst, uint spp, uint first, uint n, uint* queue, uint* countPtr, hipStream_t st);
void launch_extend(const DeviceScene& sc, PathPool pool, const uint* queue, const uint* countPtr, uint count, WaveCounters* wc, bool counters, TravAux aux, hipStream_t st, bool ranged = false);
void launch_extend_first(const PathKernelContext& k, PathPool pool, FirstVertex fv, const uint* countPtr, uint count, WaveCounters* wc, TravAux aux, hipStream_t st);
void launch_shade(const PathKernelContext& k, PathPool pool, const uint* queueIn, const uint* countInPtr, uint countIn, uint* queueOut, uint* countOutPtr,
                  ShadowQueue sq, WaveCounters* wc, uint* classScratch, uint* classCount, hipStream_t st, PathPool outPool = PathPool{},
                  const FirstVertex* fv = nullptr, const uint* inertBits = nullptr);
void launch_uncompact(PathPool in, PathPool out, const uint* countPtr, uint count, hipStream_t st);
void launch_classify(PathPool pool, const uint* queueIn, const uint* countInPtr, uint countIn, uint* classScratch, uint* classCount, hipStream_t st);
void launch_shadow(const DeviceScene& sc, PathPool pool, ShadowQueue sq, const uint* countPtr, uint count, WaveCounters* wc, bool counters, TravAux aux, hipStream_t st);
void launch_trace_pair(const DeviceScene& sc, PathPool pool, const uint* queue, const uint* extCountPtr, uint extCount, ShadowQueue sq, uint* shCountPtr, uint shCount, WaveCounters* wc, TravAux auxE, TravAux auxS, hipStream_t st);
void launch_tail(const PathKernelContext& k, PathPool pool, const uint* queueIn, const uint* countInPtr, uint countIn, uint* queueOut, uint* countOutPtr, ShadowQueue sq, WaveCounters* wc, uint maxBounces, uint deferIters , uint maxBlocks, hipStream_t st);
void launch_pass_reset(uint* passCounters, uint* nextCount, uint* shadowCount, hipStream_t st);
void launch_accumulate(PathPool pool, const uint* ownedPixels, uint numOwned, uint spp, float4* accum, uint accumCountBase, uint width, hipStream_t st);
void launch_trace_probe(const DeviceScene& sc, const float4* rays, uint n, float4* outClosest, uint* outVisible, uint* overflow, hipStream_t st);
void launch_pack(const float4* accum, const uint* ownedPixels, uint numOwned, uint width, float4* dst, hipStream_t st);
void launch_unpack(float4* accum, const uint* pixels, uint num, uint width, const float4* src, hipStream_t st);
void launch_pack_feedback(const float* fbW, const uint* fbC, const float* depth, const uint* pixels, uint num, uint width, uint* dst, hipStream_t st);
void launch_unpack_feedback(float* fbW, uint* fbC, float* depth, const uint* pixels, uint num, uint width, const uint* src, hipStream_t st);
void launch_env_cube_bake(const DeviceScene& sc, const EnvDirectionalLight* lights, uint nLights, uint2* texels, const EnvCube& cube, hipStream_t st);
void launch_env_cube_compress(uint2* texels, const EnvCube& cube, uint quality, hipStream_t st);
void launch_env_importance(const DeviceScene& sc, uint dim, uint sx, uint sy, float4* out, hipStream_t st);
void launch_bake_emissive(const DeviceScene& sc, const uint* subInstList, const uint* subInstTriOffset, uint numEmissiveSubInst, uint totalTris, uint lightBase,
                          PolymorphicLightInfo* lights, PolymorphicLightInfoEx* lightsEx, hipStream_t st);
void launch_light_weights(const PolymorphicLightInfo* lights, const PolymorphicLightInfoEx* lightsEx, uint n, float* w, const LightFrustumBoost& boost, hipStream_t st);
void launch_light_proxy_counts(const float* w, uint n, float* sum, uint budget, bool uniform, uint maxPerLight, uint* counts, const uint* usage, uint totalMaxFeedbackCount, float globalFeedbackUseWeight, hipStream_t st);
void launch_neeat_boost_weights(const float* base, const float* hist, uint nHist, uint n, float mul, float* cur, hipStream_t st);
void launch_neeat_begin(const NeeAtFrame& F, float* snapW, uint* snapC, bool preFilter, uint totalThreads, hipStream_t st);
void launch_neeat_end(const NeeAtFrame& F, hipStream_t st);
void launch_light_proxy_fill(const uint* counts, const uint* offsets, uint n, uint* proxies, uint capacity, hipStream_t st);
void launch_tonemap(const float4* accum, uint num, const ToneMapParams& p, uint* outRgba8, hipStream_t st);
void launch_average_log_luminance(const float4* accum, uint W, uint H, float* scratch, float** result, hipStream_t st);
void launch_probe(const PathKernelContext& k, int kind, const void* dIn, void* dOut, uint n, hipStream_t st);

}
```

rtxpt_amd/csrc/pt_wavefront.hip:

```cpp
#include "pt_wavefront.h"
#include "pt_traverse8.h"
#include "pt_traverse8p.h"
#include "pt_wavefront_device.h"
#include <cstdlib>
#define T8_TRAVERSE traverse8_pairs

namespace ptk {

#ifndef T8_CHUNKS_PER_WAVE_MIN
#define T8_CHUNKS_PER_WAVE_MIN 1
#endif
#ifndef T8_SHORT_TAIL_BELOW
#define T8_SHORT_TAIL_BELOW 32768u
#endif
#ifndef T8_TASK_BLOCKS_N
#define T8_TASK_BLOCKS_N 512
#endif

__global__ void __launch_bounds__(256) k_generate(PathKernelContext k, PathPool pool, const uint* __restrict__ ownedPixels, uint numOwned, uint sampleFirst, uint spp, uint first, uint n, uint* __restrict__ queue, uint* countPtr) {
    const uint t = blockIdx.x * 256u + threadIdx.x;
    if (t >= n) return;
    const uint i = first + t;
    uint px, sample; first_vertex_of(FirstVertex{ownedPixels, numOwned, sampleFirst, spp}, i, px, sample);
    PathState p = k.generate(px >> 16, px & 0xFFFFu, sample);
    store_path(pool, i, p);
    queue[t] = i;
    if (countPtr && t == 0u) atomicAdd(countPtr, n);
}

template <bool COUNT, bool RANGED, bool FIRST = false>
__device__ __forceinline__ void t8_extend_body(const DeviceScene& sc, const PathPool& pool, const uint* __restrict__ queue, const uint count, WaveCounters* wc, const TravAux& aux, const uint rpc,
                                               uint2* stack, uint* rayBuf, float2* mineUV, const uint vBlock, const uint vGrid, const FirstVertex* fv = nullptr) {
    static_assert(!FIRST || (!COUNT && !RANGED), "vertex 0 in place: composed frames only");
    Traverse8Counters ctr; t8_counters_init(ctr);
    auto fetch = [&](uint i, float3& o, float3& d, float& tmin, float& tmax, uint& startRef, float& bestT0, uint& bestPrim0) -> uint {
        if (FIRST) {
            asm volatile("" ::: "memory");
            const FirstVertexCamera fc = wc->firstCamera;
            uint px, sample; first_vertex_of(*fv, i, px, sample);
            PathKernelContext::cameraRay(fc.cam, fc.perPixelJitterAAScale, px >> 16, px & 0xFFFFu, sample, o, d);
            tmin = 0.0f; tmax = kMaxRayTravel; startRef = 0u; bestT0 = kMaxRayTravel; bestPrim0 = 0xFFFFFFFFu;
            return i;
        }
        uint p = pool.home ? i : queue[i];
        uint4 a = pool.s0[p], b = pool.s1[p];
        o = make_float3(asfloat(a.x), asfloat(a.y), asfloat(a.z)); d = make_float3(asfloat(b.x), asfloat(b.y), asfloat(b.z));
        tmin = 0.0f; tmax = kMaxRayTravel; startRef = 0u; bestT0 = kMaxRayTravel; bestPrim0 = 0xFFFFFFFFu;
        if (RANGED) { const uint4 r = pool.hit[p]; tmin = asfloat(r.x); tmax = asfloat(r.y); bestT0 = tmax; }
        return p;
    };
    auto commit = [&](uint p, const HitInfo& h) { pool.hit[p] = make_uint4(asuint(h.t), h.prim, asuint(h.u), asuint(h.v)); };
    auto publish = [&](uint p, float bestT, uint bestPrim) { aux.bestKey[p] = t8_hit_key(bestT, bestPrim); aux.resolveList[atomicAdd(&aux.counts[TRAV_RESOLVE], 1u)] = p; };
    if (COUNT) { ctr.rayIterHist = wc->rayIterHistExt; ctr.longRayCount = &wc->longRayCount; ctr.longRays = &wc->longRays[0][0]; }
    T8_TRAVERSE<false, COUNT, !RANGED, false, true>(sc, count, rpc, stack, rayBuf, mineUV, fetch, commit, publish, TravTaskOut{aux.taskQ[0], &aux.counts[0], aux.taskCap}, ctr, &wc->overflow, vBlock, vGrid);
    if (COUNT) { wave_add64(ctr.nodeVisits, &wc->nodeVisitsExt); wave_add64(ctr.triTests, &wc->triTestsExt); wave_add64(ctr.leafVisits, &wc->leafVisitsExt); wave_add64(ctr.iters, &wc->itersExt); wave_add64(ctr.leafBlocks, &wc->leafBlocksExt); if ((threadIdx.x & 63u) == 0u) atomicMax(&wc->itersMaxExt, (unsigned long long)ctr.iters);
                 if ((threadIdx.x & 63u) == 0u) for (int q = 0; q < 4; q++) atomicAdd(&wc->phaseCycExt[q], ctr.cyc[q]);
                 for (int q = 0; q < 8; q++) wave_add64(ctr.ev[q], &wc->eventsExt[q]); }
}
template <bool COUNT, bool RANGED = false>
__global__ void __launch_bounds__(T8_BLOCK, T8_EXTEND_MIN_BLOCKS) k_extend(DeviceScene sc, PathPool pool, const uint* __restrict__ queue, const uint* __restrict__ countPtr, WaveCounters* wc, TravAux aux, uint rpc) {
    __shared__ uint2 stack[T8_GROUPS_PER_BLOCK * BVH8_STACK_STRIDE];
    __shared__ uint rayBuf[T8_RAYBUF_WORDS];
    __shared__ float2 mineUV[T8_BLOCK];
    t8_extend_body<COUNT, RANGED>(sc, pool, queue, *countPtr, wc, aux, rpc, stack, rayBuf, mineUV, blockIdx.x, gridDim.x);
}

__global__ void __launch_bounds__(T8_BLOCK, T8_EXTEND_MIN_BLOCKS) k_extend_first(DeviceScene sc, PathPool pool, FirstVertex fv, const uint* __restrict__ countPtr, WaveCounters* wc, TravAux aux, uint rpc) {
    __shared__ uint2 stack[T8_GROUPS_PER_BLOCK * BVH8_STACK_STRIDE];
    __shared__ uint rayBuf[T8_RAYBUF_WORDS];
    __shared__ float2 mineUV[T8_BLOCK];
    t8_extend_body<false, false, true>(sc, pool, nullptr, *countPtr, wc, aux, rpc, stack, rayBuf, mineUV, blockIdx.x, gridDim.x, &fv);
}

__global__ void __launch_bounds__(256) k_first_split_rays(PathKernelContext k, PathPool pool, FirstVertex fv, TravAux aux) {
    const uint n = aux.counts[TRAV_RESOLVE];
    for (uint i = blockIdx.x * 256u + threadIdx.x; i < n; i += gridDim.x * 256u) {
        const uint p = aux.resolveList[i];
        uint px, sample; first_vertex_of(fv, p, px, sample);
        float3 o, d; k.computeCameraRay(px >> 16, px & 0xFFFFu, sample, o, d);
        pool.s0[p] = make_uint4(asuint(o.x), asuint(o.y), asuint(o.z), px); pool.s1[p] = make_uint4(asuint(d.x), asuint(d.y), asuint(d.z), asuint(0.0f));
    }
}

#ifndef T8_TASK_SPREAD
#define T8_TASK_SPREAD 1
#endif
__device__ __forceinline__ uint t8_tasks_per_chunk(uint count) { return (!T8_TASK_SPREAD || count > T8_GROUPS_PER_WAVE * 4u * T8_TASK_BLOCKS_N || T8_GROUPS_PER_WAVE > T8_CHUNK) ? T8_CHUNK : T8_GROUPS_PER_WAVE; }
template <int STAGE, bool FINAL>
__device__ __forceinline__ void t8_extend_tasks_body(const DeviceScene& sc, const PathPool& pool, WaveCounters* wc, const TravAux& aux, uint2* stack, uint* rayBuf, const uint vBlock, const uint vGrid) {
    constexpr int IN = STAGE & 1;
    uint count = aux.counts[STAGE]; if (count > aux.taskCap) count = aux.taskCap;
    if (count == 0u) return;
    const TravTask* tasks = aux.taskQ[IN];
    const uint real = t8_tasks_per_chunk(count), per = (count + real - 1u) / real;
    Traverse8Counters ctr; t8_counters_init(ctr);
    auto fetch = [&](uint i, float3& o, float3& d, float& tmin, float& tmax, uint& startRef, float& bestT0, uint& bestPrim0) -> uint {
        const uint lane = i % T8_CHUNK, j = lane * per + i / T8_CHUNK;
        const bool pad = lane >= real || j >= count;
        TravTask t = tasks[pad ? 0u : j];
        if (pad) t.tbits = 0x7F800000u;
        uint4 a = pool.s0[t.tag], b = pool.s1[t.tag];
        o = make_float3(asfloat(a.x), asfloat(a.y), asfloat(a.z)); d = make_float3(asfloat(b.x), asfloat(b.y), asfloat(b.z));
        unsigned long long key = aux.bestKey[t.tag];
        tmin = 0.0f; tmax = kMaxRayTravel; bestT0 = __uint_as_float((uint)(key >> 32)); bestPrim0 = (uint)key;
        startRef = (__uint_as_float(t.tbits) <= bestT0) ? t.ref : BVH_EMPTY;
        return t.tag;
    };
    auto commit = [&](uint p, const HitInfo& h) { atomicMin(&aux.bestKey[p], t8_hit_key(h.t, h.prim)); };
    auto publish = [&](uint p, float bestT, uint bestPrim) { if (bestPrim != 0xFFFFFFFFu) atomicMin(&aux.bestKey[p], t8_hit_key(bestT, bestPrim)); };
    T8_TRAVERSE<false, false, true, true, !FINAL>(sc, per * T8_CHUNK, T8_CHUNK, stack, rayBuf, nullptr, fetch, commit, publish, TravTaskOut{aux.taskQ[IN ^ 1], &aux.counts[FINAL ? STAGE : STAGE + 1], FINAL ? 0u : aux.taskCap}, ctr, &wc->overflow, vBlock, vGrid);
}
template <int STAGE, bool FINAL = (STAGE == 3)>
__global__ void __launch_bounds__(T8_BLOCK, T8_EXTEND_MIN_BLOCKS) k_extend_tasks(DeviceScene sc, PathPool pool, WaveCounters* wc, TravAux aux) {
    __shared__ uint2 stack[T8_GROUPS_PER_BLOCK * BVH8_STACK_STRIDE];
    __shared__ uint rayBuf[T8_TASKBUF_WORDS];
    t8_extend_tasks_body<STAGE, FINAL>(sc, pool, wc, aux, stack, rayBuf, blockIdx.x, gridDim.x);
}

__device__ __forceinline__ void t8_resolve_extend_body(const DeviceScene& sc, const PathPool& pool, const TravAux& aux, const uint vBlock, const uint vGrid) {
    const uint n = aux.counts[TRAV_RESOLVE];
    for (uint i = vBlock * 256u + threadIdx.x; i < n; i += vGrid * 256u) {
        uint p = aux.resolveList[i];
        unsigned long long key = aux.bestKey[p];
        uint prim = (uint)key;
        uint4 out = make_uint4((uint)(key >> 32), prim, 0u, 0u);
        if (prim != 0xFFFFFFFFu) {
            uint4 a = pool.s0[p], b = pool.s1[p];
            float3 o = make_float3(asfloat(a.x), asfloat(a.y), asfloat(a.z)), d = make_float3(asfloat(b.x), asfloat(b.y), asfloat(b.z));
            float t, u = 0.f, v = 0.f;
            const TriRecord tr = sc.tris[aux.primToSlot[prim]]; (void)intersect_tri_wt(tri_v0(tr), tri_v1(tr), tri_v2(tr), o, d, 0.0f, kMaxRayTravel, t, u, v);
            out.z = asuint(u); out.w = asuint(v);
        }
        pool.hit[p] = out;
    }
}
__global__ void __launch_bounds__(256) k_resolve_extend(DeviceScene sc, PathPool pool, TravAux aux) { t8_resolve_extend_body(sc, pool, aux, blockIdx.x, gridDim.x); }

#ifndef PT_SHADE_BLOCK
#define PT_SHADE_BLOCK 256
#endif
#ifndef PT_SHADE_MIN_BLOCKS
#define PT_SHADE_MIN_BLOCKS 1
#endif
#ifndef PT_SHADE_PROBE
#define PT_SHADE_PROBE 0
#endif
#ifndef PT_SHADE_CLASSES
#define PT_SHADE_CLASSES 1
#endif

#define PT_CLASSIFY_ITEMS 4u
template <bool UNIFORM = false, bool DROP = false>
__global__ void __launch_bounds__(1024) k_classify(PathPool pool, const uint* __restrict__ queueIn, const uint* __restrict__ countInPtr, uint* __restrict__ classQ, uint* __restrict__ classCount, uint uniformFlags,
                                                   const uint* __restrict__ inertBits, uint nestedDielectricsQuality) {
    static_assert(!(UNIFORM && DROP), "vertex 0 has no terminating paths");
    __shared__ uint waveCnt[PT_CLASSIFY_ITEMS][16][4]; __shared__ uint blockBase[3];
    const uint count = *countInPtr, wave = threadIdx.x >> 6, lane = threadIdx.x & 63u;
    uint p[PT_CLASSIFY_ITEMS], cls[PT_CLASSIFY_ITEMS]; unsigned long long mine[PT_CLASSIFY_ITEMS];
#pragma unroll
    for (uint j = 0; j < PT_CLASSIFY_ITEMS; j++) {
        const uint i = (blockIdx.x * PT_CLASSIFY_ITEMS + j) * 1024u + threadIdx.x;
        p[j] = 0u; cls[j] = 4u;
        if (i < count) {
            p[j] = pool.home ? i : queueIn[i];
            const uint prim = reinterpret_cast<const uint*>(pool.hit)[4u * (size_t)p[j] + 1u], flags = UNIFORM ? uniformFlags : reinterpret_cast<const uint*>(pool.s4)[4u * (size_t)p[j] + 2u];
            cls[j] = (prim == 0xFFFFFFFFu) ? 2u : (((flags >> kVertexIndexBitCount) & PF_terminateAtNextBounce) ? 1u : 0u);
            if (DROP && cls[j] == 1u && inert_when_terminal(inert_bits_at(inertBits, prim), nestedDielectricsQuality)) cls[j] = 3u;
        }
        const unsigned long long m0 = __builtin_amdgcn_ballot_w64(cls[j] == 0u), m1 = __builtin_amdgcn_ballot_w64(cls[j] == 1u), m2 = __builtin_amdgcn_ballot_w64(cls[j] == 2u);
        if (lane == 0u) { waveCnt[j][wave][0] = (uint)__popcll(m0); waveCnt[j][wave][1] = (uint)__popcll(m1); waveCnt[j][wave][2] = (uint)__popcll(m2); }
        if (DROP) { const unsigned long long m3 = __builtin_amdgcn_ballot_w64(cls[j] == 3u); if (lane == 0u) waveCnt[j][wave][3] = (uint)__popcll(m3); }
        mine[j] = cls[j] == 0u ? m0 : (cls[j] == 1u ? m1 : m2);
    }
    __syncthreads();
    if (threadIdx.x < 3u) {
        uint tot = 0;
        for (uint j = 0; j < PT_CLASSIFY_ITEMS; j++) for (uint w = 0; w < 16u; w++) { const uint c = waveCnt[j][w][threadIdx.x]; waveCnt[j][w][threadIdx.x] = tot; tot += c; }
        blockBase[threadIdx.x] = tot ? atomicAdd(&classCount[threadIdx.x], tot) : 0u;
    } else if (DROP && threadIdx.x == 3u) {
        uint tot = 0;
        for (uint j = 0; j < PT_CLASSIFY_ITEMS; j++) for (uint w = 0; w < 16u; w++) tot += waveCnt[j][w][3];
        if (tot) atomicAdd(&classCount[3], tot);
    }
    __syncthreads();
#pragma unroll
    for (uint j = 0; j < PT_CLASSIFY_ITEMS; j++) {
        if (cls[j] > 2u) continue;
        const uint rank = blockBase[cls[j]] + waveCnt[j][wave][cls[j]] + (uint)__popcll(mine[j] & ((1ull << lane) - 1ull));
        classQ[cls[j] == 0u ? rank : (cls[j] == 1u ? count - 1u - rank : count + rank)] = p[j];
    }
}

template <bool MULTI, class PKC, bool NEEAT, bool COMPACT = false, bool FIRST = false>
__global__ void __launch_bounds__(PT_SHADE_BLOCK, PT_SHADE_MIN_BLOCKS) k_shade(PKC k, PathPool pool, const uint* __restrict__ queueIn, const uint* __restrict__ countInPtr,
                                               uint* __restrict__ queueOut, uint* countOutPtr, ShadowQueue sq, WaveCounters* wc, const uint* __restrict__ classCount, PathPool outPool, FirstVertex fv) {
    static_assert(!FIRST || (COMPACT && !MULTI && !NEEAT), "vertex 0 in place: the compacted pool of a composed frame");
    static_assert(!COMPACT || !PT_SHADE_PROBE, "the PT_SHADE_PROBE timing builds do not know the compacted pool: take the COMPACT launch out of launch_shade and run with MI355PT_COMPACT_POOL=0");
    const uint count = *countInPtr;
    uint i = blockIdx.x * (uint)PT_SHADE_BLOCK + threadIdx.x;
    bool inRange = i < count;
    bool alive = false; bool isHit = false; uint p = 0, hp = 0;
    ShadowRequest req; req.valid = false;
    PathState cpath;
    if (COMPACT) __builtin_memset(&cpath, 0, sizeof(cpath));
    if (inRange) {
        if (classCount) {
            const uint nGo = classCount[0], nEnd = classCount[1];
            inRange = i < nGo + nEnd + classCount[2];
            p = inRange ? queueIn[i < nGo ? i : (i < nGo + nEnd ? count - 1u - (i - nGo) : count + (i - nGo - nEnd))] : 0u;
        } else p = COMPACT ? i : queueIn[i];
    }
    if (inRange) {
        hp = (COMPACT && !FIRST) ? pool.home[p] : p;
        uint4 hr = pool.hit[p];
        HitInfo h; h.t = asfloat(hr.x); h.prim = hr.y; h.u = asfloat(hr.z); h.v = asfloat(hr.w);
#if PT_SHADE_PROBE
        PathState path = load_path(pool, p);
#if PT_SHADE_PROBE == 1
        if (h.prim != 0xFFFFFFFFu) { isHit = true; path.sceneLength += h.t; } path.terminate();
#elif PT_SHADE_PROBE == 2
        if (h.prim != 0xFFFFFFFFu) { isHit = true; SurfaceData sfd = k.loadSurface(h.prim, h.u, h.v, path.dir, path.rayCone); path.origin = sfd.shadingData.posW + sfd.shadingData.N * sfd.bsdf.data.roughness + sfd.bsdf.data.diffuse + sfd.shadingData.T; } path.terminate();
#endif
        store_path(pool, p, path);
        alive = path.isActive();
// ... 356 lines not shown
    case 0: { const float* p = in + 3 * i; int fn = (int)p[0]; float x = p[1], y = p[2]; float r;
        switch (fn) { case 0: r = dm_sin(x); break; case 1: r = dm_cos(x); break; case 2: r = dm_exp2(x); break; case 3: r = dm_log2(x); break;
                      case 4: r = dm_atan2(y, x); break; case 5: r = dm_pow(x, y); break; case 6: r = FastACos(x); break; default: r = FastSqrt(x); break; }
        out[i] = r; } break;
    case 1: { float x = in[i]; uint hbits = f32tof16(x); out[2 * i] = asfloat(hbits); out[2 * i + 1] = f16tof32(hbits); } break;
    case 2: { const uint* p = reinterpret_cast<const uint*>(in) + 6 * i;
        SampleGeneratorVertexBase vb = SampleGeneratorVertexBase::make(p[0], p[1], p[2]);
        uint cnt = p[5] > 8 ? 8 : p[5];
        if (p[4] == 0) { float4 v = SampleSequenceGenerator::Generate(cnt, vb, p[3]); out[8 * i] = v.x; out[8 * i + 1] = v.y; out[8 * i + 2] = v.z; out[8 * i + 3] = v.w; }
        else if (p[4] == 1) { float4 v = UniformSampleSequenceGenerator::Generate(cnt, vb, p[3]); out[8 * i] = v.x; out[8 * i + 1] = v.y; out[8 * i + 2] = v.z; out[8 * i + 3] = v.w; }
        else if (p[4] == 2) { UniformSampleSequenceGenerator g = UniformSampleSequenceGenerator::make(vb, p[3]); for (uint j = 0; j < cnt; j++) out[8 * i + j] = sampleNext1D(g); }
        else { SampleSequenceGenerator g = SampleSequenceGenerator::make(vb, p[3], p[4] == 4); for (uint j = 0; j < cnt; j++) out[8 * i + j] = sampleNext1D(g); } } break;
    case 3: { const float* p = in + 24 * i;
        ShadingData sd; __builtin_memset(&sd, 0, sizeof(sd));
        sd.N = make_float3(0, 0, 1); sd.T = make_float3(1, 0, 0); sd.B = make_float3(0, 1, 0); sd.V = make_float3(p[16], p[17], p[18]);
        sd.faceNCorrected = sd.N; sd.vertexN = sd.N; sd.frontFacing = true; sd.mtl = MaterialHeader::make(); sd.mtl.setActiveLobes(Lobe_All); sd.mtl.setThinSurface(p[14] != 0.f);
        StandardBSDF b; b.diffuseModel = (int)p[15];
        b.data.diffuse = make_float3(p[0], p[1], p[2]); b.data.specular = make_float3(p[3], p[4], p[5]); b.data.roughness = p[6]; b.data.metallic = p[7];
        b.data.transmission = make_float3(p[8], p[9], p[10]); b.data.diffuseTransmission = p[11]; b.data.specularTransmission = p[12]; b.data.eta = p[13];
        float* o = out + 10 * i;
        if (p[22] == 0.f) { float3 wo = make_float3(p[19], p[20], p[21]); float4 e = b.eval(sd, wo); o[0] = e.x; o[1] = e.y; o[2] = e.z; o[3] = e.w; o[4] = b.evalPdf(sd, wo); o[5] = (float)b.getLobes(); o[6] = o[7] = o[8] = o[9] = 0.f; }
        else { BSDFSample s; __builtin_memset(&s, 0, sizeof(s)); bool v = b.sample(sd, make_float4(p[19], p[20], p[21], 0), s);
               o[0] = s.wo.x; o[1] = s.wo.y; o[2] = s.wo.z; o[3] = s.pdf; o[4] = s.weight.x; o[5] = s.weight.y; o[6] = s.weight.z; o[7] = (float)s.lobe; o[8] = s.lobeP; o[9] = v ? 1.f : 0.f; } } break;
    case 4: { const uint* p = reinterpret_cast<const uint*>(in) + 3 * i;
        PathState ps = k.generate(p[0], p[1], p[2]);
        out[6 * i] = ps.origin.x; out[6 * i + 1] = ps.origin.y; out[6 * i + 2] = ps.origin.z; out[6 * i + 3] = ps.dir.x; out[6 * i + 4] = ps.dir.y; out[6 * i + 5] = ps.dir.z; } break;
    case 5: { const float* a = in + 9 * i + 1; int fn = (int)in[9 * i]; float* o = out + 4 * i; o[0] = o[1] = o[2] = o[3] = 0.f;
        switch (fn) {
        case 0: o[0] = evalFresnelSchlick(a[0], a[1], a[2]); break;
        case 1: { float3 r = evalFresnelSchlick(make_float3(a[0], a[1], a[2]), a[3], a[4]); o[0] = r.x; o[1] = r.y; o[2] = r.z; } break;
        case 2: { float ct = 0.f; o[0] = evalFresnelDielectric(a[0], a[1], ct); o[1] = ct; } break;
        case 3: o[0] = evalNdfGGX(a[0], a[1]); break;
        case 4: o[0] = evalPdfGGX_BVNDF(a[0], make_float3(a[1], a[2], a[3]), make_float3(a[4], a[5], a[6])); break;
        case 5: { float3 r = sampleGGX_BVNDF(a[0], make_float3(a[1], a[2], a[3]), make_float2(a[4], a[5])); o[0] = r.x; o[1] = r.y; o[2] = r.z; } break;
        case 6: o[0] = evalLambdaGGX(a[0], a[1]); break;
        case 7: o[0] = evalMaskingSmithGGXCorrelated(a[0], a[1], a[2]); break;
        case 8: { float2 r = ndir_to_oct_equal_area_unorm(make_float3(a[0], a[1], a[2])); o[0] = r.x; o[1] = r.y; } break;
        case 9: { float3 r = oct_to_ndir_equal_area_unorm(make_float2(a[0], a[1])); o[0] = r.x; o[1] = r.y; o[2] = r.z; } break;
        case 10: { float2 r = sample_disk(make_float2(a[0], a[1])); o[0] = r.x; o[1] = r.y; } break;
        case 11: { float2 r = sample_disk_concentric(make_float2(a[0], a[1])); o[0] = r.x; o[1] = r.y; } break;
        case 12: { float pdf = 0.f; float3 r = sample_cosine_hemisphere_concentric(make_float2(a[0], a[1]), pdf); o[0] = r.x; o[1] = r.y; o[2] = r.z; o[3] = pdf; } break;
        case 13: { float3 r = perp_stark(make_float3(a[0], a[1], a[2])); o[0] = r.x; o[1] = r.y; o[2] = r.z; } break;
        case 14: { float3 r = ComputeRayOrigin(make_float3(a[0], a[1], a[2]), make_float3(a[3], a[4], a[5])); o[0] = r.x; o[1] = r.y; o[2] = r.z; } break;
        case 15: o[0] = FastSqrt(a[0]); break;
        case 16: o[0] = FastACos(a[0]); break;
        case 17: o[0] = ComputeRayConeSpreadAngleExpansionByScatterPDF(a[0], a[1]); break;
        case 18: o[0] = ComputeNewScatterFireflyFilterK<LPOps<false>>(a[0], a[1], a[2]); break;
        case 19: { float3 r = FireflyFilter<LPOps<false>>(make_float3(a[0], a[1], a[2]), a[3], a[4]); o[0] = r.x; o[1] = r.y; o[2] = r.z; } break;
        case 20: o[0] = FireflyFilterShort(a[0], a[1], a[2]); break;
        case 21: o[0] = ComputeLowGrazingAngleFalloff(make_float3(a[0], a[1], a[2]), make_float3(a[3], a[4], a[5]), a[6], a[7]); break;
        default: break;
        } } break;
    case 6: { const uint* a = reinterpret_cast<const uint*>(in) + 19 * i + 1; const uint lk = reinterpret_cast<const uint*>(in)[19 * i]; uint* o = reinterpret_cast<uint*>(out) + 12 * i;
        for (int q = 0; q < 12; q++) o[q] = 0u;
        const float3x4 I = {{1, 0, 0, 0, 0, 1, 0, 0, 0, 0, 1, 0}};
        auto info = [&](const uint* w) { PolymorphicLightInfoFull li; __builtin_memset(&li, 0, sizeof(li));
            li.Base.Center = make_float3(asfloat(w[0]), asfloat(w[1]), asfloat(w[2])); li.Base.ColorTypeAndFlags = w[3]; li.Base.Direction1 = w[4]; li.Base.Direction2 = w[5]; li.Base.Scalars = w[6]; li.Base.LogRadiance = w[7];
            li.Extended.IesProfileIndex = w[8]; li.Extended.PrimaryAxis = w[9]; li.Extended.CosConeAngleAndSoftness = w[10]; li.Extended.UniqueID = w[11]; return li; };
        if (lk == 0u) { PolymorphicLightInfo b; __builtin_memset(&b, 0, sizeof(b)); PackLightColor(make_float3(asfloat(a[0]), asfloat(a[1]), asfloat(a[2])), b); float3 c = UnpackLightColor(b);
            o[0] = b.ColorTypeAndFlags; o[1] = b.LogRadiance; o[2] = asuint(c.x); o[3] = asuint(c.y); o[4] = asuint(c.z); }
        else if (lk == 1u) { TriangleLight t; t.base = make_float3(asfloat(a[0]), asfloat(a[1]), asfloat(a[2])); t.edge1 = make_float3(asfloat(a[3]), asfloat(a[4]), asfloat(a[5])); t.edge2 = make_float3(asfloat(a[6]), asfloat(a[7]), asfloat(a[8]));
            t.radiance = make_float3(asfloat(a[9]), asfloat(a[10]), asfloat(a[11])); t.normal = make_float3(0.f); t.surfaceArea = 0;
            PolymorphicLightInfoFull li = t.Store(7u);
            o[0] = asuint(li.Base.Center.x); o[1] = asuint(li.Base.Center.y); o[2] = asuint(li.Base.Center.z); o[3] = li.Base.ColorTypeAndFlags; o[4] = li.Base.Direction1; o[5] = li.Base.Direction2; o[6] = li.Base.Scalars; o[7] = li.Base.LogRadiance;
            o[8] = li.Extended.IesProfileIndex; o[9] = li.Extended.PrimaryAxis; o[10] = li.Extended.CosConeAngleAndSoftness; o[11] = li.Extended.UniqueID; }
        else if (lk == 2u) { PolymorphicLightInfoFull li = info(a);
            PolymorphicLightSample sm = PolymorphicLight_CalcSample(li, make_float2(asfloat(a[12]), asfloat(a[13])), make_float3(asfloat(a[14]), asfloat(a[15]), asfloat(a[16])), I);
            o[0] = asuint(sm.Position.x); o[1] = asuint(sm.Position.y); o[2] = asuint(sm.Position.z); o[3] = asuint(sm.Normal.x); o[4] = asuint(sm.Normal.y); o[5] = asuint(sm.Normal.z);
            o[6] = asuint(sm.Radiance.x); o[7] = asuint(sm.Radiance.y); o[8] = asuint(sm.Radiance.z); o[9] = asuint(sm.SolidAnglePdf); o[10] = sm.LightSampleableByBSDF ? 1u : 0u; o[11] = asuint(PolymorphicLight_GetPower(li)); }
        else if (lk == 3u) { TriangleLight t = TriangleLight::Create(info(a));
            o[0] = asuint(t.CalcSolidAnglePdfForMIS(make_float3(asfloat(a[12]), asfloat(a[13]), asfloat(a[14])), make_float3(asfloat(a[15]), asfloat(a[16]), asfloat(a[17])))); }
        else { uint pk = NDirToOctUnorm32(make_float3(asfloat(a[0]), asfloat(a[1]), asfloat(a[2]))); float3 d = OctToNDirUnorm32(pk); o[0] = pk; o[1] = asuint(d.x); o[2] = asuint(d.y); o[3] = asuint(d.z); }
        } break;
    case 8: { const float* a = in + 8 * i; uint* o = reinterpret_cast<uint*>(out) + 45 * i;
        RayCone rc = RayCone::make(a[6], a[7]);
        auto emit = [&](const SurfaceData& q) {
            const ShadingData& s = q.shadingData; const StandardBSDFData& b = q.bsdf.data;
            auto put3 = [&](float3 v) { *o++ = asuint(v.x); *o++ = asuint(v.y); *o++ = asuint(v.z); };
            put3(s.posW); put3(s.faceNCorrected); put3(s.V); put3(s.N); put3(s.T); put3(s.B); put3(s.vertexN);
            *o++ = s.frontFacing ? 1u : 0u; *o++ = s.mtl.packedData; *o++ = s.materialID; *o++ = asuint(s.IoR); *o++ = asuint(s.shadowNoLFadeout); put3(s.emission);
            put3(b.diffuse); *o++ = asuint(b.roughness); put3(b.specular); *o++ = asuint(b.metallic); put3(b.transmission);
            *o++ = asuint(b.diffuseTransmission); *o++ = asuint(b.specularTransmission); *o++ = asuint(b.eta); *o++ = asuint(q.interiorIoR); *o++ = q.neeTriangleLightIndex; };
        if (k.S.useFp16Types) { PathKernelContextT<true> k16; __builtin_memcpy(&k16, &k, sizeof(k16)); emit(k16.loadSurface(asuint(a[0]), a[1], a[2], make_float3(a[3], a[4], a[5]), rc)); }
        else emit(k.loadSurface(asuint(a[0]), a[1], a[2], make_float3(a[3], a[4], a[5]), rc));
        } break;
    case 7: { const float* a = in + 4 * i; const int op = (int)a[0]; typedef LPOps<true> H; float r = 0.f;
        switch (op) { case 0: r = H::r(a[1]); break; case 1: r = H::add(H::r(a[1]), H::r(a[2])); break; case 2: r = H::sub(H::r(a[1]), H::r(a[2])); break; case 3: r = H::mul(H::r(a[1]), H::r(a[2])); break;
                      case 4: r = H::div(H::r(a[1]), H::r(a[2])); break; case 5: r = H::lerp(H::r(a[1]), H::r(a[2]), H::r(a[3])); break;
                      case 7: r = H::r(a[1] * a[2]); break; case 8: r = H::r(H::r(a[1]) * a[2]); break; case 9: r = H::r(a[1] + a[2]); break; case 10: r = H::r(a[1] / a[2]); break;
                      default: r = H::average3(make_float3(H::r(a[1]), H::r(a[2]), H::r(a[3]))); break; }
        out[i] = r; } break;
    case 10: { const uint* a = reinterpret_cast<const uint*>(in) + 3 * i; uint* o = reinterpret_cast<uint*>(out) + 2 * i;
        const uint slot = k.sc.primToSlot[a[0]]; const TriRecord tr = k.sc.tris[slot];
        const bool solid = !(tr.flags & 1u) || alpha_test_slot(k.sc, slot, asfloat(a[1]), asfloat(a[2]));
        o[0] = solid ? 1u : 0u; o[1] = (!(tr.flags & 1u) || (!(tr.flags & 2u) && solid)) ? 1u : 0u; } break;
    case 9: { const float* a = in + 4 * i; float* o = out + 3 * i;
        float3 r = k.sc.envEnabled ? env_eval_local(k.sc, make_float3(a[0], a[1], a[2]), a[3]) : make_float3(0.f);
        o[0] = r.x; o[1] = r.y; o[2] = r.z; } break;
    case 11: { const uint* a = reinterpret_cast<const uint*>(in) + 8 * i; const float2 uv = make_float2(asfloat(a[2]), asfloat(a[3])); float4 r;
        if (a[0] == 0u) r = k.sampleTexture(a[1], asfloat(a[4]), uv);
        else if (a[0] == 1u) r = sample_bilinear(k.sc, k.sc.textures[a[1]], a[4], uv);
        else r = sample_grad_anisotropic(k.sc, k.sc.textures[a[1]], uv, make_float2(asfloat(a[4]), asfloat(a[5])), make_float2(asfloat(a[6]), asfloat(a[7])));
        out[4 * i] = r.x; out[4 * i + 1] = r.y; out[4 * i + 2] = r.z; out[4 * i + 3] = r.w; } break;
    default: break;
    }
}
#endif

#ifndef T8_ADAPTIVE_CHUNKS
#define T8_ADAPTIVE_CHUNKS 1
#endif
static inline uint rays_per_chunk(uint count) {
    if (!T8_ADAPTIVE_CHUNKS) return T8_CHUNK;
    const uint resident = 256u * 4u * 8u;
    const uint step = T8_GROUPS_PER_WAVE;
    uint r = ((count + resident - 1u) / resident + step - 1u) / step * step;
    return r < step ? (step > T8_CHUNK ? T8_CHUNK : step) : (r > T8_CHUNK ? T8_CHUNK : r);
}
static inline uint grid_for(uint count, uint block, uint maxBlocks) { uint g = (count + block - 1) / block; if (g < 1) g = 1; if (g > maxBlocks) g = maxBlocks; return g; }

__global__ void __launch_bounds__(256) k_tonemap(const float4* __restrict__ accum, uint num, ToneMapParams p, uint* __restrict__ out) {
    uint i = blockIdx.x * 256u + threadIdx.x;
    if (i < num) out[i] = tm_pixel(p, accum[i]);
}
void launch_tonemap(const float4* accum, uint num, const ToneMapParams& p, uint* outRgba8, hipStream_t st) {
    hipLaunchKernelGGL(k_tonemap, dim3((num + 255) / 256), dim3(256), 0, st, accum, num, p, outRgba8);
}
__global__ void __launch_bounds__(256) k_log_luminance(const float4* __restrict__ accum, uint W, uint H, uint LW, uint LH, float* __restrict__ out) {
    uint i = blockIdx.x * 256u + threadIdx.x;
    if (i < LW * LH) out[i] = tm_log_luminance_texel(accum, W, H, LW, LH, i % LW, i / LW);
}
__global__ void __launch_bounds__(256) k_luminance_mip(const float* __restrict__ src, uint w, uint h, uint ow, uint oh, float* __restrict__ dst) {
    uint i = blockIdx.x * 256u + threadIdx.x;
    if (i < ow * oh) dst[i] = tm_mip_texel(src, w, h, i % ow, i / ow);
}
void launch_average_log_luminance(const float4* accum, uint W, uint H, float* scratch, float** result, hipStream_t st) {
    uint w = tm_pow2_floor(W), h = tm_pow2_floor(H);
    float* a = scratch; float* b = scratch + (size_t)w * h;
    hipLaunchKernelGGL(k_log_luminance, dim3((w * h + 255) / 256), dim3(256), 0, st, accum, W, H, w, h, a);
    while (w > 1u || h > 1u) {
        uint ow = w > 1u ? w / 2u : 1u, oh = h > 1u ? h / 2u : 1u;
        hipLaunchKernelGGL(k_luminance_mip, dim3((ow * oh + 255) / 256), dim3(256), 0, st, a, w, h, ow, oh, b);
        float* t = a; a = b; b = t; w = ow; h = oh;
    }
    *result = a;
}
void launch_generate(const PathKernelContext& k, PathPool pool, const uint* ownedPixels, uint numOwned, uint sampleFirst, uint spp, uint first, uint n, uint* queue, uint* countPtr, hipStream_t st) {
    if (n) hipLaunchKernelGGL(k_generate, dim3((n + 255) / 256), dim3(256), 0, st, k, pool, ownedPixels, numOwned, sampleFirst, spp, first, n, queue, countPtr);
}
static const uint T8_TASK_BLOCKS = T8_TASK_BLOCKS_N, T8_RESOLVE_BLOCKS = 256;
static const uint T8_SWEEP_BLOCKS = 2048;
static inline uint shadow_resolve_grid(uint count) { const uint g = grid_for(count, 256u, T8_SWEEP_BLOCKS); return g < T8_RESOLVE_BLOCKS ? T8_RESOLVE_BLOCKS : g; }
static void launch_extend_stragglers(const DeviceScene& sc, PathPool pool, uint count, WaveCounters* wc, TravAux aux, hipStream_t st);
void launch_extend_first(const PathKernelContext& k, PathPool pool, FirstVertex fv, const uint* countPtr, uint count, WaveCounters* wc, TravAux aux, hipStream_t st) {
    const uint rpc = rays_per_chunk(count);
    const uint g = grid_for(count, (T8_BLOCK / 64u) * rpc * T8_CHUNKS_PER_WAVE_MIN, (aux.maxBlocks && aux.maxBlocks < T8_MAX_BLOCKS) ? aux.maxBlocks : T8_MAX_BLOCKS);
    hipLaunchKernelGGL(k_extend_first, dim3(g), dim3(T8_BLOCK), 0, st, k.sc, pool, fv, countPtr, wc, aux, rpc);
    hipLaunchKernelGGL(k_first_split_rays, dim3(T8_RESOLVE_BLOCKS), dim3(256), 0, st, k, pool, fv, aux);
    launch_extend_stragglers(k.sc, pool, count, wc, aux, st);
}
void launch_extend(const DeviceScene& sc, PathPool pool, const uint* queue, const uint* countPtr, uint count, WaveCounters* wc, bool counters, TravAux aux, hipStream_t st, bool ranged) {
    const uint rpc = rays_per_chunk(count);
    uint g = grid_for(count, (T8_BLOCK / 64u) * rpc * T8_CHUNKS_PER_WAVE_MIN, (aux.maxBlocks && aux.maxBlocks < T8_MAX_BLOCKS) ? aux.maxBlocks : T8_MAX_BLOCKS);
    if (ranged) { if (counters) hipLaunchKernelGGL((k_extend<true, true>), dim3(g), dim3(T8_BLOCK), 0, st, sc, pool, queue, countPtr, wc, aux, rpc);
                  else hipLaunchKernelGGL((k_extend<false, true>), dim3(g), dim3(T8_BLOCK), 0, st, sc, pool, queue, countPtr, wc, aux, rpc); }
    else if (counters) hipLaunchKernelGGL((k_extend<true>), dim3(g), dim3(T8_BLOCK), 0, st, sc, pool, queue, countPtr, wc, aux, rpc);
    else hipLaunchKernelGGL((k_extend<false>), dim3(g), dim3(T8_BLOCK), 0, st, sc, pool, queue, countPtr, wc, aux, rpc);
    launch_extend_stragglers(sc, pool, count, wc, aux, st);
}
static void launch_extend_stragglers(const DeviceScene& sc, PathPool pool, uint count, WaveCounters* wc, TravAux aux, hipStream_t st) {
    if (count <= T8_SHORT_TAIL_BELOW) {
        hipLaunchKernelGGL((k_extend_tasks<0>), dim3(T8_TASK_BLOCKS), dim3(T8_BLOCK), 0, st, sc, pool, wc, aux);
        hipLaunchKernelGGL((k_extend_tasks<1, true>), dim3(T8_TASK_BLOCKS), dim3(T8_BLOCK), 0, st, sc, pool, wc, aux);
        hipLaunchKernelGGL(k_resolve_extend, dim3(T8_RESOLVE_BLOCKS), dim3(256), 0, st, sc, pool, aux);
        return;
    }
    hipLaunchKernelGGL((k_extend_tasks<0>), dim3(T8_TASK_BLOCKS), dim3(T8_BLOCK), 0, st, sc, pool, wc, aux);
    hipLaunchKernelGGL((k_extend_tasks<1>), dim3(T8_TASK_BLOCKS), dim3(T8_BLOCK), 0, st, sc, pool, wc, aux);
    hipLaunchKernelGGL((k_extend_tasks<2>), dim3(T8_TASK_BLOCKS), dim3(T8_BLOCK), 0, st, sc, pool, wc, aux);
    hipLaunchKernelGGL((k_extend_tasks<3>), dim3(T8_TASK_BLOCKS), dim3(T8_BLOCK), 0, st, sc, pool, wc, aux);
    hipLaunchKernelGGL(k_resolve_extend, dim3(T8_RESOLVE_BLOCKS), dim3(256), 0, st, sc, pool, aux);
}
void launch_trace_pair(const DeviceScene& sc, PathPool pool, const uint* queue, const uint* extCountPtr, uint extCount, ShadowQueue sq, uint* shCountPtr, uint shCount, WaveCounters* wc, TravAux auxE, TravAux auxS, hipStream_t st) {
    const uint rpc = rays_per_chunk(extCount + shCount);
    const uint bound = (auxE.maxBlocks && auxE.maxBlocks < T8_MAX_BLOCKS) ? auxE.maxBlocks : T8_MAX_BLOCKS;
    uint gE = grid_for(extCount, (T8_BLOCK / 64u) * rpc * T8_CHUNKS_PER_WAVE_MIN, bound), gS = grid_for(shCount, (T8_BLOCK / 64u) * rpc * T8_CHUNKS_PER_WAVE_MIN, bound);
    if (gE + gS > bound) {
        uint s = (uint)(((unsigned long long)bound * shCount + (extCount + shCount) / 2u) / (extCount + shCount)); if (s < 1u) s = 1u; if (s > bound - 1u) s = bound - 1u;
        if (s > gS) s = gS;
        uint e = bound - s; if (e > gE) { e = gE; s = (bound - e < gS) ? bound - e : gS; }
        gE = e; gS = s;
    }
    hipLaunchKernelGGL(k_trace_pair, dim3(gE + gS), dim3(T8_BLOCK), 0, st, sc, pool, queue, extCountPtr, sq, shCountPtr, wc, auxE, auxS, rpc, rpc, gE);
    const dim3 tg(2u * T8_TASK_BLOCKS), tb(T8_BLOCK);
    if (extCount <= T8_SHORT_TAIL_BELOW && shCount <= T8_SHORT_TAIL_BELOW) {
        hipLaunchKernelGGL((k_tasks_pair<0>), tg, tb, 0, st, sc, pool, sq, wc, auxE, auxS);
        hipLaunchKernelGGL((k_tasks_pair<1, true>), tg, tb, 0, st, sc, pool, sq, wc, auxE, auxS);
    } else {
        hipLaunchKernelGGL((k_tasks_pair<0>), tg, tb, 0, st, sc, pool, sq, wc, auxE, auxS);
        hipLaunchKernelGGL((k_tasks_pair<1>), tg, tb, 0, st, sc, pool, sq, wc, auxE, auxS);
        hipLaunchKernelGGL((k_tasks_pair<2>), tg, tb, 0, st, sc, pool, sq, wc, auxE, auxS);
        hipLaunchKernelGGL((k_tasks_pair<3>), tg, tb, 0, st, sc, pool, sq, wc, auxE, auxS);
    }
    hipLaunchKernelGGL(k_resolve_pair, dim3(T8_RESOLVE_BLOCKS + shadow_resolve_grid(shCount)), dim3(256), 0, st, sc, pool, sq, auxE, auxS, shCountPtr, shCount, T8_RESOLVE_BLOCKS);
}
void launch_classify(PathPool pool, const uint* queueIn, const uint* countInPtr, uint countIn, uint* classScratch, uint* classCount, hipStream_t st) {
    hipLaunchKernelGGL((k_classify<false>), dim3((countIn + 1024u * PT_CLASSIFY_ITEMS - 1u) / (1024u * PT_CLASSIFY_ITEMS)), dim3(1024), 0, st, pool, queueIn, countInPtr, classScratch, classCount, 0u, (const uint*)nullptr, 0u);
}
void launch_shade(const PathKernelContext& k, PathPool pool, const uint* queueIn, const uint* countInPtr, uint countIn, uint* queueOut, uint* countOutPtr, ShadowQueue sq, WaveCounters* wc,
                  uint* classScratch, uint* classCount, hipStream_t st, PathPool outPool, const FirstVertex* fv, const uint* inertBits) {
    const FirstVertex fv0 = fv ? *fv : FirstVertex{nullptr, 0u, 0u, 0u};
    const dim3 g((countIn + PT_SHADE_BLOCK - 1) / PT_SHADE_BLOCK), b(PT_SHADE_BLOCK);
    const bool neeat = k.sc.lights.LocalSamplingBuffer != nullptr || k.sc.lights.TemporalFeedbackRequired != 0u;
    if (PT_SHADE_CLASSES && classScratch) {
        const dim3 cg((countIn + 1024u * PT_CLASSIFY_ITEMS - 1u) / (1024u * PT_CLASSIFY_ITEMS));
        const bool drop = inertBits && !neeat && k.sc.lights.DepthExport == nullptr;
        if (fv) hipLaunchKernelGGL((k_classify<true>), cg, dim3(1024), 0, st, pool, queueIn, countInPtr, classScratch, classCount, k.generateState(0u, 0u, 0u).flagsAndVertexIndex, (const uint*)nullptr, 0u);
        else if (drop) hipLaunchKernelGGL((k_classify<false, true>), cg, dim3(1024), 0, st, pool, queueIn, countInPtr, classScratch, classCount, 0u, inertBits, (uint)k.S.nestedDielectricsQuality);
        else hipLaunchKernelGGL((k_classify<false>), cg, dim3(1024), 0, st, pool, queueIn, countInPtr, classScratch, classCount, 0u, (const uint*)nullptr, 0u);
        queueIn = classScratch;
    } else classCount = nullptr;
#define PT_LAUNCH_SHADE(MULTI, PKC, CTX) do { if (neeat) hipLaunchKernelGGL((k_shade<MULTI, PKC, true>), g, b, 0, st, CTX, pool, queueIn, countInPtr, queueOut, countOutPtr, sq, wc, classCount, outPool, fv0); \
                                              else if (pool.home && !MULTI && fv) hipLaunchKernelGGL((k_shade<false, PKC, false, true, true>), g, b, 0, st, CTX, pool, queueIn, countInPtr, queueOut, countOutPtr, sq, wc, classCount, outPool, fv0); \
                                              else if (pool.home && !MULTI) hipLaunchKernelGGL((k_shade<false, PKC, false, true>), g, b, 0, st, CTX, pool, queueIn, countInPtr, queueOut, countOutPtr, sq, wc, classCount, outPool, fv0); \
                                              else hipLaunchKernelGGL((k_shade<MULTI, PKC, false>), g, b, 0, st, CTX, pool, queueIn, countInPtr, queueOut, countOutPtr, sq, wc, classCount, outPool, fv0); } while (0)
    if (k.S.useFp16Types) {
        static_assert(sizeof(PathKernelContextT<true>) == sizeof(PathKernelContext), "the two lp builds share one context layout");
        PathKernelContextT<true> k16; __builtin_memcpy(&k16, &k, sizeof(k16));
        if (sq.group) PT_LAUNCH_SHADE(true, PathKernelContextT<true>, k16); else PT_LAUNCH_SHADE(false, PathKernelContextT<true>, k16);
    } else {
        if (sq.group) PT_LAUNCH_SHADE(true, PathKernelContext, k); else PT_LAUNCH_SHADE(false, PathKernelContext, k);
    }
#undef PT_LAUNCH_SHADE
}
void launch_shadow(const DeviceScene& sc, PathPool pool, ShadowQueue sq, const uint* countPtr, uint count, WaveCounters* wc, bool counters, TravAux aux, hipStream_t st) {
    const uint rpc = rays_per_chunk(count);
    uint g = grid_for(count, (T8_BLOCK / 64u) * rpc * T8_CHUNKS_PER_WAVE_MIN, (aux.maxBlocks && aux.maxBlocks < T8_MAX_BLOCKS) ? aux.maxBlocks : T8_MAX_BLOCKS);
    if (counters && !sq.group) hipLaunchKernelGGL((k_shadow<true>), dim3(g), dim3(T8_BLOCK), 0, st, sc, sq, countPtr, wc, aux, rpc);
    else hipLaunchKernelGGL((k_shadow<false>), dim3(g), dim3(T8_BLOCK), 0, st, sc, sq, countPtr, wc, aux, rpc);
    hipLaunchKernelGGL((k_shadow_tasks<0>), dim3(T8_TASK_BLOCKS), dim3(T8_BLOCK), 0, st, sc, sq, wc, aux);
    if (count <= T8_SHORT_TAIL_BELOW) hipLaunchKernelGGL((k_shadow_tasks<1, true>), dim3(T8_TASK_BLOCKS), dim3(T8_BLOCK), 0, st, sc, sq, wc, aux);
    else {
    hipLaunchKernelGGL((k_shadow_tasks<1>), dim3(T8_TASK_BLOCKS), dim3(T8_BLOCK), 0, st, sc, sq, wc, aux);
    hipLaunchKernelGGL((k_shadow_tasks<2>), dim3(T8_TASK_BLOCKS), dim3(T8_BLOCK), 0, st, sc, sq, wc, aux);
    hipLaunchKernelGGL((k_shadow_tasks<3>), dim3(T8_TASK_BLOCKS), dim3(T8_BLOCK), 0, st, sc, sq, wc, aux);
    }
    if (sq.group) hipLaunchKernelGGL((k_resolve_shadow<true>), dim3(T8_RESOLVE_BLOCKS), dim3(256), 0, st, pool, sq, aux, 0u);
    else hipLaunchKernelGGL((k_resolve_shadow<false>), dim3(shadow_resolve_grid(count)), dim3(256), 0, st, pool, sq, aux, count);
    if (sq.group) hipLaunchKernelGGL(k_resolve_nee, dim3(grid_for(count / sq.group, 256, 4096)), dim3(256), 0, st, pool, sq, countPtr);
}
__global__ void __launch_bounds__(64) k_pass_begin(uint* __restrict__ passCounters, uint* __restrict__ nextCount, uint* __restrict__ shadowCount) {
    if (threadIdx.x < PASS_COUNTERS) passCounters[threadIdx.x] = 0u;
    if (threadIdx.x == 32u) *nextCount = 0u;
    if (threadIdx.x == 33u && shadowCount) *shadowCount = 0u;
}
void launch_pass_reset(uint* passCounters, uint* nextCount, uint* shadowCount, hipStream_t st) { static_assert(PASS_COUNTERS <= 32u, "k_pass_begin"); hipLaunchKernelGGL(k_pass_begin, dim3(1), dim3(64), 0, st, passCounters, nextCount, shadowCount); }
__global__ void __launch_bounds__(256) k_uncompact(PathPool in, PathPool out, const uint* __restrict__ countPtr) {
    const uint i = blockIdx.x * 256u + threadIdx.x;
    if (i >= *countPtr) return;
    const uint hp = in.home[i];
    out.s0[hp] = in.s0[i]; out.s1[hp] = in.s1[i]; out.s3[hp] = in.s3[i]; out.s4[hp] = in.s4[i];
}
void launch_uncompact(PathPool in, PathPool out, const uint* countPtr, uint count, hipStream_t st) {
    if (count) hipLaunchKernelGGL(k_uncompact, dim3((count + 255u) / 256u), dim3(256), 0, st, in, out, countPtr);
}
void launch_accumulate(PathPool pool, const uint* ownedPixels, uint numOwned, uint spp, float4* accum, uint accumCountBase, uint width, hipStream_t st) {
    hipLaunchKernelGGL(k_accumulate, dim3((numOwned + 255) / 256), dim3(256), 0, st, pool, ownedPixels, numOwned, spp, accum, accumCountBase, width);
}
void launch_trace_probe(const DeviceScene& sc, const float4* rays, uint n, float4* outClosest, uint* outVisible, uint* overflow, hipStream_t st) {
    hipLaunchKernelGGL(k_trace_probe, dim3(grid_for(n, T8_BLOCK, T8_MAX_BLOCKS)), dim3(T8_BLOCK), 0, st, sc, rays, n, outClosest, outVisible, overflow);
}
__global__ void __launch_bounds__(256) k_pack_feedback(const float* __restrict__ fbW, const uint* __restrict__ fbC, const float* __restrict__ depth, const uint* __restrict__ pixels, uint num, uint width, uint* __restrict__ dst) {
    uint i = blockIdx.x * 256u + threadIdx.x; if (i >= num) return;
    const uint px = pixels[i], slot = (px & 0xFFFFu) * width + (px >> 16);
    dst[3u * i] = __float_as_uint(fbW[slot]); dst[3u * i + 1u] = fbC[slot]; dst[3u * i + 2u] = depth ? __float_as_uint(depth[slot]) : 0u;
}
__global__ void __launch_bounds__(256) k_unpack_feedback(float* __restrict__ fbW, uint* __restrict__ fbC, float* __restrict__ depth, const uint* __restrict__ pixels, uint num, uint width, const uint* __restrict__ src) {
    uint i = blockIdx.x * 256u + threadIdx.x; if (i >= num) return;
    const uint px = pixels[i], slot = (px & 0xFFFFu) * width + (px >> 16);
    fbW[slot] = __uint_as_float(src[3u * i]); fbC[slot] = src[3u * i + 1u]; if (depth) depth[slot] = __uint_as_float(src[3u * i + 2u]);
}
void launch_pack_feedback(const float* fbW, const uint* fbC, const float* depth, const uint* pixels, uint num, uint width, uint* dst, hipStream_t st) {
    if (num) hipLaunchKernelGGL(k_pack_feedback, dim3((num + 255) / 256), dim3(256), 0, st, fbW, fbC, depth, pixels, num, width, dst);
}
void launch_unpack_feedback(float* fbW, uint* fbC, float* depth, const uint* pixels, uint num, uint width, const uint* src, hipStream_t st) {
    if (num) hipLaunchKernelGGL(k_unpack_feedback, dim3((num + 255) / 256), dim3(256), 0, st, fbW, fbC, depth, pixels, num, width, src);
}
void launch_pack(const float4* accum, const uint* pixels, uint num, uint width, float4* dst, hipStream_t st) {
    hipLaunchKernelGGL(k_pack, dim3((num + 255) / 256), dim3(256), 0, st, accum, pixels, num, width, dst);
}
void launch_unpack(float4* accum, const uint* pixels, uint num, uint width, const float4* src, hipStream_t st) {
    hipLaunchKernelGGL(k_unpack, dim3((num + 255) / 256), dim3(256), 0, st, accum, pixels, num, width, src);
}
void launch_env_importance(const DeviceScene& sc, uint dim, uint sx, uint sy, float4* out, hipStream_t st) {
    hipLaunchKernelGGL(k_env_importance, dim3((dim * dim + 255) / 256), dim3(256), 0, st, sc, dim, sx, sy, out);
}
__global__ void __launch_bounds__(256) k_light_weights(const PolymorphicLightInfo* __restrict__ lights, const PolymorphicLightInfoEx* __restrict__ lightsEx, uint n, float* __restrict__ w, LightFrustumBoost boost) {
    uint i = blockIdx.x * 256u + threadIdx.x; if (i >= n) return;
    PolymorphicLightInfoFull lf; lf.Base = lights[i]; lf.Extended = lightsEx[i];
    float wt = dm_pow(PolymorphicLight_GetPower(lf), 0.8f);
    if (!(wt >= 1e-8f)) wt = 0.f;
    w[i] = light_importance_frustum_boost(boost, lf, wt);
}
__global__ void __launch_bounds__(256) k_light_weight_sum(const float* __restrict__ w, uint n, float* __restrict__ sum) {
    __shared__ float stage[256];
    float s = 0.f;
    for (uint base = 0; base < n; base += 256u) {
        const uint i = base + threadIdx.x;
        stage[threadIdx.x] = (i < n) ? w[i] : 0.f;
// ... 132 lines not shown
```

Before: 1913 Mrays/s.

## Trace camera rays as wave-coherent packets with leftover handoff to per-ray traversal

```diff
diff --git a/rtxpt_amd/csrc/pt_api.hip b/rtxpt_amd/csrc/pt_api.hip
--- a/rtxpt_amd/csrc/pt_api.hip
+++ b/rtxpt_amd/csrc/pt_api.hip
@@ -533,6 +533,9 @@
     { const char* e = getenv("MI355PT_TAIL_PATHS"); if (e) c->tailBelow = (uint)strtoul(e, nullptr, 10); }
     { const char* e = getenv("MI355PT_COMPACT_POOL"); if (e) c->compactPool = atoi(e) != 0; }
     { const char* e = getenv("MI355PT_FIRST_VERTEX_IN_PLACE"); if (e) c->firstVertexInPlace = atoi(e) != 0; }
+    { const char* e = getenv("MI355PT_FIRST_VERTEX_PACKETS"); if (e) c->firstVertexPackets = atoi(e) != 0; }
+    { const char* e = getenv("MI355PT_PACKET_STEP_CAP"); if (e) c->packetStepCap = (uint)strtoul(e, nullptr, 10); }
+    { const char* e = getenv("MI355PT_PACKET_STACK"); if (e) c->packetStack = (uint)strtoul(e, nullptr, 10); }
     { const char* e = getenv("MI355PT_FUSED_TRAVERSAL"); if (e) c->fusedTraversal = (uint)strtoul(e, nullptr, 10); }
     { const char* e = getenv("MI355PT_DROP_INERT_TERMINAL"); if (e) c->dropInertTerminal = atoi(e) != 0; }
     { const char* e = getenv("MI355PT_TAIL_DEFER"); if (e) c->tailDefer = (uint)strtoul(e, nullptr, 10); }
@@ -556,7 +559,7 @@
     c->dIndices.free(); c->dNormals.free(); c->dTangents.free(); c->dProxyCounters.free(); c->dProxyIndices.free(); c->dEnvLookup.free(); c->dOwned.free(); c->dQueue[0].free(); c->dQueue[1].free();
     c->dPrevPositions.free(); c->dPrevInstances.free(); c->dEmissiveList.free(); c->dEmissiveOffsets.free(); c->dPositions.free(); c->dUvs.free(); c->dGeometries.free(); c->dInstances.free(); c->dSubInstances.free(); c->dSubInstToInstGeom.free();
     c->dPrimInfo.free(); c->dShadeTris.free(); c->dInertBits.free(); c->dAlphaPlanes.free(); c->dAlphaPool.free(); c->dMaterials.free(); c->dTexInfos.free(); c->dTexels.free(); c->dEnvCube.free(); c->dEnvCubeSource.free(); c->dEnvImageCube.free(); c->dEnvDirLights.free(); c->dLights.free(); c->dLightsEx.free(); c->dS0.free(); c->dS1.free(); c->dS2.free(); c->dS3.free(); c->dS4.free();
-    c->dHit.free(); c->dS0b.free(); c->dS1b.free(); c->dS3b.free(); c->dS4b.free(); c->dHitb.free(); c->dSq0.free(); c->dSq1.free(); c->dSq2.free(); c->dAccum.free(); c->dScratch4.free(); c->dCounters.free(); c->dTravSpill.free(); c->dTaskQ.free(); c->dTravCounts.free(); c->dResolveList.free(); c->dBestKey.free(); c->dResolveListSh.free(); c->dBestKeySh.free(); c->dTaskQSh.free();
+    c->dHit.free(); c->dS0b.free(); c->dS1b.free(); c->dS3b.free(); c->dS4b.free(); c->dHitb.free(); c->dSq0.free(); c->dSq1.free(); c->dSq2.free(); c->dAccum.free(); c->dScratch4.free(); c->dCounters.free(); c->dTravSpill.free(); c->dTaskQ.free(); c->dTravCounts.free(); c->dResolveList.free(); c->dFirstLeftover.free(); c->dBestKey.free(); c->dResolveListSh.free(); c->dBestKeySh.free(); c->dTaskQSh.free();
     for (uint b = 1; b < PT_PIPELINE_BATCHES; b++) (void)hipStreamDestroy(c->streams[b]);
     (void)hipStreamDestroy(c->stream); (void)hipHostFree(c->hostCounters);
     delete c;
diff --git a/rtxpt_amd/csrc/pt_context.h b/rtxpt_amd/csrc/pt_context.h
--- a/rtxpt_amd/csrc/pt_context.h
+++ b/rtxpt_amd/csrc/pt_context.h
@@ -68,6 +68,9 @@
 #ifndef PT_FIRST_VERTEX_IN_PLACE
 #define PT_FIRST_VERTEX_IN_PLACE 1
 #endif
+#ifndef PT_FIRST_VERTEX_PACKETS
+#define PT_FIRST_VERTEX_PACKETS 1
+#endif
 #ifndef PT_DROP_INERT_TERMINAL
 #define PT_DROP_INERT_TERMINAL 1
 #endif
@@ -83,6 +86,7 @@
     int device = 0; hipStream_t stream = nullptr; uint shardRank = 0, shardCount = 1;
     hipStream_t streams[PT_PIPELINE_BATCHES] = {}; WaveCounters* hostCounters = nullptr; bool serialKernels = false;
     uint tailBelow = PT_TAIL_PATHS, tailDefer = 0, fusedTraversal = PT_FUSED_TRAVERSAL; bool compactPool = PT_COMPACT_POOL != 0, firstVertexInPlace = PT_FIRST_VERTEX_IN_PLACE != 0;
+    bool firstVertexPackets = PT_FIRST_VERTEX_PACKETS != 0; uint packetStepCap = 0, packetStack = 0; DevBuf<uint> dFirstLeftover;
     bool dropInertTerminal = PT_DROP_INERT_TERMINAL != 0; unsigned long long droppedTerminal = 0;
     std::string lastError;
     std::vector<uint> indices; std::vector<float> positions; std::vector<ptk::float2> uvs; std::vector<uint> normals, tangents;
diff --git a/rtxpt_amd/csrc/pt_frame.hip b/rtxpt_amd/csrc/pt_frame.hip
--- a/rtxpt_amd/csrc/pt_frame.hip
+++ b/rtxpt_amd/csrc/pt_frame.hip
@@ -134,6 +134,7 @@
     uint pendingShadow = 0; TravAux auxSh;
     PathPool poolSet[2]; uint set = 0; bool compact = false;
     bool firstInPlace = false;
+    FirstPackets packets = {nullptr, nullptr, 0u, 0u, 0u};
     bool timed = false; Events marks; size_t t0 = 0, t1 = 0;
     struct Span { size_t a, b; int kind; uint items; }; std::vector<Span> spans;
     size_t mark() { return timed ? marks.mark(st) : 0; }
@@ -174,7 +175,7 @@
         const bool neeatShade = c->dsc.lights.LocalSamplingBuffer != nullptr || c->dsc.lights.TemporalFeedbackRequired != 0u;
         if (composed && c->compactPool && !neeatShade && !feedback) {
             int32_t r = enable_compact_pool(); if (r != PT_OK) return r;
-            if (c->firstVertexInPlace) enable_first_vertex_in_place();
+            if (c->firstVertexInPlace) { enable_first_vertex_in_place(); if (c->firstVertexPackets) { r = enable_first_vertex_packets(); if (r != PT_OK) return r; } }
         }
         return PT_OK;
     }
@@ -204,6 +205,15 @@
             RenderBatch& t = B[b]; t.firstInPlace = t.compact && !(tailBelow && t.total <= tailBelow);
             t.hwc->firstCamera.cam = t.k.cam; t.hwc->firstCamera.perPixelJitterAAScale = t.k.S.perPixelJitterAAScale;
         }
+    }
+    int32_t enable_first_vertex_packets() {
+        PT_CHECK_HIP(c, c->dFirstLeftover.resize(c->poolCapacity));
+        for (uint b = 0; b < numBatches; b++) {
+            RenderBatch& t = B[b]; if (!t.firstInPlace) continue;
+            t.packets = FirstPackets{c->dFirstLeftover.p + t.base, t.aux.counts + PASS_LEFTOVER, t.total,
+                                     c->packetStepCap ? c->packetStepCap : (uint)T8_PACKET_STEP_CAP, c->packetStack ? c->packetStack : (uint)T8_PACKET_STACK};
+        }
+        return PT_OK;
     }
     int32_t start() {
         for (uint b = 0; b < numBatches; b++) {
@@ -225,7 +235,7 @@
         const uint* countIn = &t.wc->extendCount[t.cur];
         const bool vertex0 = t.firstInPlace && t.iterations == 0u;
         const FirstVertex fv{c->dOwned.p + t.pixFirst, t.numPix, first, count};
-        if (vertex0) launch_extend_first(t.k, pin, fv, countIn, t.active, t.wc, t.aux, t.st);
+        if (vertex0) launch_extend_first(t.k, pin, fv, countIn, t.active, t.wc, t.aux, t.packets, t.st);
         else if (t.pendingShadow) {
             launch_trace_pair(t.sc, pin, t.queue[t.cur], countIn, t.active, t.sq, &t.wc->shadowCount, t.pendingShadow, t.wc, t.aux, t.auxSh, t.st);
             t.pendingShadow = 0;
@@ -268,6 +278,8 @@
             uint pc[PASS_COUNTERS]; PT_CHECK_HIP(c, hipMemcpy(pc, t.aux.counts, sizeof(pc), hipMemcpyDeviceToHost));
             fprintf(stderr, "[pass log]   b%u pass %u: %u paths -> extend splits %u / %u / %u / %u sub-trees, %u rays resolved; %u visibility rays next\n",
                     b, t.iterations, t.active, pc[0], pc[1], pc[2], pc[3], pc[TRAV_RESOLVE], nShadow);
+            if (t.packets.leftover && t.iterations == 0u)
+                fprintf(stderr, "[pass log]   b%u pass 0: %u of %u camera rays left over by the packets (step cap %u, stack %u)\n", b, pc[PASS_LEFTOVER], t.active, t.packets.stepCap, t.packets.stackBound);
             if (t.active >= PT_CLASSIFY_FROM)
                 fprintf(stderr, "[pass log]   b%u pass %u: classes %u continuing / %u terminating / %u misses, %u inert terminating hits dropped\n",
                         b, t.iterations, pc[PASS_CLASS_OFFSET], pc[PASS_CLASS_OFFSET + 1], pc[PASS_CLASS_OFFSET + 2], pc[PASS_CLASS_OFFSET + 3]);
diff --git a/rtxpt_amd/csrc/pt_traverse8k.h b/rtxpt_amd/csrc/pt_traverse8k.h
--- /dev/null
+++ b/rtxpt_amd/csrc/pt_traverse8k.h
@@ -0,0 +1,190 @@
+#pragma once
+#include "pt_traverse8p.h"
+#include "pt_wavefront.h"
+
+namespace ptk {
+
+
+#define DPP_ROW_ROR(n) (0x120 + (n))
+__device__ __forceinline__ uint t8k_min(uint a, uint b) { return a < b ? a : b; }
+__device__ __forceinline__ uint t8k_max(uint a, uint b) { return a > b ? a : b; }
+__device__ __forceinline__ uint t8k_uniform(uint v) { return (uint)__builtin_amdgcn_readfirstlane((int)v); }
+
+template <class Ray, class Dst>
+__device__ __forceinline__ void traverse8_packets(const DeviceScene& sc, const uint count, uint2* stackBase, float2* mineUV, Ray form, Dst commit, const FirstPackets pk, uint* overflowFlag) {
+    static_assert(T8_LANES == 2u, "traverse8_packets keeps the lane-pair layout");
+    const uint lane = threadIdx.x & 63u, h = lane & 1u;
+    const uint wavesPerBlock = T8_BLOCK / 64u;
+    const uint waveId = t8k_uniform(blockIdx.x * wavesPerBlock + (threadIdx.x >> 6)), numWaves = t8k_uniform(gridDim.x * wavesPerBlock);
+    uint2* stack = stackBase + t8k_uniform(threadIdx.x >> 6) * T8_PACKET_STACK;
+    const char* nodesBase = reinterpret_cast<const char*>(sc.nodes8);
+    const char* trisBase = reinterpret_cast<const char*>(sc.tris);
+    const uint laneChildOff = 16u + 48u * h, laneTriOff = 48u * h;
+    const uint INF_BITS = 0x7F800000u;
+    const float tmin = 0.f, tmax = kMaxRayTravel;
+    const uint kSel = (lane >> 1) & 3u, myChild = 4u * h + kSel;
+    const uint stepCap = t8k_uniform(pk.stepCap), stackBound = t8k_uniform(pk.stackBound < T8_PACKET_STACK ? pk.stackBound : T8_PACKET_STACK);
+    const uint numPackets = (count + T8_PACKET_RAYS - 1u) / T8_PACKET_RAYS;
+
+    for (uint p = waveId; p < numPackets; p += numWaves) {
+        const uint i0 = p * T8_PACKET_RAYS, i = i0 + (lane >> 1);
+        const bool valid = i < count;
+        float3 o; float Sx, Sy, ix, iy, iz; uint axes, selN, selF;
+        {   float3 rd; form(valid ? i : count - 1u, o, rd);
+            ix = t8_rcp_dir(rd.x); iy = t8_rcp_dir(rd.y); iz = t8_rcp_dir(rd.z);
+            const float adx = fabsf(rd.x), ady = fabsf(rd.y), adz = fabsf(rd.z);
+            const bool rk2 = adz > adx && adz > ady, rk1 = !rk2 && ady > adx;
+            const float rSz = rk2 ? iz : (rk1 ? iy : ix);
+            Sx = (rk2 ? rd.x : (rk1 ? rd.z : rd.y)) * rSz; Sy = (rk2 ? rd.y : (rk1 ? rd.x : rd.z)) * rSz;
+            axes = rk2 ? (0u | (16u << 8) | (32u << 16)) : (rk1 ? (32u | (0u << 8) | (16u << 16)) : (16u | (32u << 8) | (0u << 16)));
+            const uint nxb = ix < 0.f ? 3u : 0u, fxb = ix < 0.f ? 0u : 3u, nyb = iy < 0.f ? 4u : 1u, fyb = iy < 0.f ? 1u : 4u, nzb = iz < 0.f ? 5u : 2u, fzb = iz < 0.f ? 2u : 5u;
+            selN = nxb | (nyb << 8) | (nzb << 16) | (fxb << 24); selF = fyb | (fzb << 8);
+        }
+        float bestT = valid ? tmax : -1.0f; uint bestPrim = 0xFFFFFFFFu, minePrim = 0xFFFFFFFFu;
+        uint cur = sc.rootIsValid ? 0u : BVH_EMPTY, sp = 0u, steps = 0u, maxBest = __float_as_uint(tmax);
+        bool handOff = false;
+
+        for (;;) {
+            if (cur == BVH_EMPTY) {
+                while (sp > 0u) {
+                    sp--;
+                    const uint2 e = stack[sp];
+                    const uint er = t8k_uniform(e.x), et = t8k_uniform(e.y);
+                    if (__uint_as_float(et) <= __uint_as_float(maxBest)) { cur = er; break; }
+                }
+                if (cur == BVH_EMPTY) break;
+            }
+            if (++steps > stepCap) { handOff = true; break; }
+
+            if (!(cur & BVH_LEAF_BIT)) {
+                const uint nodeOff = cur * 128u;
+                const u32x4 hdr = *reinterpret_cast<const u32x4*>(nodesBase + nodeOff);
+                const u32x4 c0 = *reinterpret_cast<const u32x4*>(nodesBase + (nodeOff + laneChildOff));
+                const u32x4 c1 = *reinterpret_cast<const u32x4*>(nodesBase + (nodeOff + laneChildOff + 16u));
+                const u32x4 c2 = *reinterpret_cast<const u32x4*>(nodesBase + (nodeOff + laneChildOff + 32u));
+                const f32x4 scl = *reinterpret_cast<const f32x4*>(nodesBase + (nodeOff + 112u));
+                const float nx = __uint_as_float(hdr.x), ny = __uint_as_float(hdr.y), nz = __uint_as_float(hdr.z);
+                const float sx = scl.x, sy = scl.y, sz = scl.z;
+                auto slab = [&](uint q0, uint q1, float& tn, float& tf) {
+                    const uint N = __builtin_amdgcn_perm(q1, q0, selN), F = __builtin_amdgcn_perm(q1, q0, selF);
+                    f32x2 px = __builtin_elementwise_fma((f32x2){(float)(N & 0xFFu), (float)(N >> 24)}, (f32x2){sx, sx}, (f32x2){nx, nx});
+                    f32x2 py = __builtin_elementwise_fma((f32x2){(float)((N >> 8) & 0xFFu), (float)(F & 0xFFu)}, (f32x2){sy, sy}, (f32x2){ny, ny});
+                    f32x2 pz = __builtin_elementwise_fma((f32x2){(float)((N >> 16) & 0xFFu), (float)((F >> 8) & 0xFFu)}, (f32x2){sz, sz}, (f32x2){nz, nz});
+                    f32x2 tx = (px - (f32x2){o.x, o.x}) * (f32x2){ix, ix}, ty = (py - (f32x2){o.y, o.y}) * (f32x2){iy, iy}, tz = (pz - (f32x2){o.z, o.z}) * (f32x2){iz, iz};
+                    tn = fmaxf(fmaxf(tx.x, ty.x), fmaxf(tz.x, tmin));
+                    tf = fminf(fminf(tx.y, ty.y), fminf(tz.y, bestT));
+                };
+                const uint ref[4] = {c0.x, c0.w, c1.z, c2.y};
+                uint key[4];
+                {   float tn, tf;
+                    slab(c0.y, c0.z, tn, tf); key[0] = T8_HIT(ref[0], tn, tf) ? (__float_as_uint(tn) & 0x7FFFFFF8u) : INF_BITS;
+                    slab(c1.x, c1.y, tn, tf); key[1] = T8_HIT(ref[1], tn, tf) ? (__float_as_uint(tn) & 0x7FFFFFF8u) : INF_BITS;
+                    slab(c1.w, c2.x, tn, tf); key[2] = T8_HIT(ref[2], tn, tf) ? (__float_as_uint(tn) & 0x7FFFFFF8u) : INF_BITS;
+                    slab(c2.z, c2.w, tn, tf); key[3] = T8_HIT(ref[3], tn, tf) ? (__float_as_uint(tn) & 0x7FFFFFF8u) : INF_BITS;
+                }
+#pragma unroll
+                for (int k = 0; k < 4; k++) {
+                    key[k] = t8k_min(key[k], dpp_u<DPP_QP_XOR2>(key[k]));
+                    key[k] = t8k_min(key[k], dpp_u<DPP_ROW_ROR(4)>(key[k]));
+                    key[k] = t8k_min(key[k], dpp_u<DPP_ROW_ROR(8)>(key[k]));
+                }
+                uint mk = kSel == 0u ? key[0] : (kSel == 1u ? key[1] : (kSel == 2u ? key[2] : key[3]));
+                const uint mref = kSel == 0u ? ref[0] : (kSel == 1u ? ref[1] : (kSel == 2u ? ref[2] : ref[3]));
+                {   auto r = __builtin_amdgcn_permlane16_swap(mk, mk, false, false); mk = t8k_min(r[0], r[1]); }
+                {   auto r = __builtin_amdgcn_permlane32_swap(mk, mk, false, false); mk = t8k_min(r[0], r[1]); }
+                const bool hitC = mk < INF_BITS && mref != BVH_EMPTY;
+                mk |= myChild;
+                uint rank = 0u;
+                rank += (dpp_u<DPP_ROW_ROR(1)>(mk) < mk) ? 1u : 0u; rank += (dpp_u<DPP_ROW_ROR(2)>(mk) < mk) ? 1u : 0u; rank += (dpp_u<DPP_ROW_ROR(3)>(mk) < mk) ? 1u : 0u;
+                rank += (dpp_u<DPP_ROW_ROR(4)>(mk) < mk) ? 1u : 0u; rank += (dpp_u<DPP_ROW_ROR(5)>(mk) < mk) ? 1u : 0u; rank += (dpp_u<DPP_ROW_ROR(6)>(mk) < mk) ? 1u : 0u;
+                rank += (dpp_u<DPP_ROW_ROR(7)>(mk) < mk) ? 1u : 0u;
+                const uint hitMask = (uint)t8_ballot(hitC) & 0xFFu;
+                uint next = BVH_EMPTY;
+                if (hitMask) {
+                    const uint nhit = (uint)__popc(hitMask);
+                    const uint nearMask = (uint)t8_ballot(hitC && rank == 0u) & 0xFFu;
+                    next = (uint)__builtin_amdgcn_readlane((int)mref, (int)(__ffs((int)nearMask) - 1));
+                    if (nhit > 1u) {
+                        if (sp + nhit - 1u > stackBound) { handOff = true; break; }
+                        if (lane < 8u && hitC && rank > 0u) stack[sp + (nhit - 1u - rank)] = make_uint2(mref, mk & ~7u);
+                        sp += nhit - 1u;
+                    }
+                }
+                cur = next;
+            } else {
+                const uint cnt = (cur & 7u) + 1u;
+                const uint slot0 = (cur & 0x7FFFFFFFu) >> 3;
+                const uint triOff0 = slot0 * 48u + laneTriOff;
+                float lt = __uint_as_float(INF_BITS), lu = 0.f, lv = 0.f; uint lp = 0xFFFFFFFFu;
+                const uint gx = axes & 0xFFu, gy = (axes >> 8) & 0xFFu, gz = axes >> 16;
+                const bool k2 = gz == 32u, k1 = gz == 16u;
+                const float okx = k2 ? o.x : (k1 ? o.z : o.y), oky = k2 ? o.y : (k1 ? o.x : o.z), okz = k2 ? o.z : (k1 ? o.y : o.x);
+                const float Sz = k2 ? iz : (k1 ? iy : ix);
+#pragma unroll 1
+                for (uint r = 0; r < T8_LEAF_ROUNDS; r++) {
+                    const bool doit = valid && (h + T8_LANES * r) < cnt;
+                    if (r > 0u && t8_ballot(doit) == 0ull) break;
+                    if (doit) {
+                        const uint toff = triOff0 + (T8_LANES * 48u) * r;
+                        struct __attribute__((packed, aligned(4))) f32x3p { float x, y, z; };
+                        const f32x3p g0 = *reinterpret_cast<const f32x3p*>(trisBase + (toff + gx)), g1 = *reinterpret_cast<const f32x3p*>(trisBase + (toff + gy)), g2 = *reinterpret_cast<const f32x3p*>(trisBase + (toff + gz));
+                        const f32x2 ABkz = (f32x2){g2.x, g2.y} - (f32x2){okz, okz}; const float Ckz = g2.z - okz;
+                        const f32x2 ABx = __builtin_elementwise_fma((f32x2){-Sx, -Sx}, ABkz, (f32x2){g0.x, g0.y} - (f32x2){okx, okx}), ABy = __builtin_elementwise_fma((f32x2){-Sy, -Sy}, ABkz, (f32x2){g1.x, g1.y} - (f32x2){oky, oky});
+                        const float Cx = fmaf(-Sx, Ckz, g0.z - okx), Cy = fmaf(-Sy, Ckz, g1.z - oky);
+                        const float Ax = ABx.x, Bx = ABx.y, Ay = ABy.x, By = ABy.y, Akz = ABkz.x, Bkz = ABkz.y;
+                        const f32x2 m1 = ABx * (f32x2){Cy, Cy}, m2 = ABy * (f32x2){Cx, Cx};
+                        float V = m1.x - m2.x, U = m2.y - m1.y, W = Bx * Ay - By * Ax;
+                        if (U == 0.0f || V == 0.0f || W == 0.0f) {
+                            if (U == 0.0f) U = fmaf(Cx, By, -(Cx * By)) - fmaf(Cy, Bx, -(Cy * Bx));
+                            if (V == 0.0f) V = fmaf(Ax, Cy, -(Ax * Cy)) - fmaf(Ay, Cx, -(Ay * Cx));
+                            if (W == 0.0f) W = fmaf(Bx, Ay, -(Bx * Ay)) - fmaf(By, Ax, -(By * Ax));
+                        }
+                        const float det = (U + V) + W;
+                        const bool inside = (bool)(((int)(fminf(U, fminf(V, W)) >= 0.0f) | (int)(fmaxf(U, fmaxf(V, W)) <= 0.0f)) & (int)(det != 0.0f));
+                        if (inside) {
+                            const float T = fmaf(W, Sz * Ckz, fmaf(V, Sz * Bkz, U * (Sz * Akz)));
+                            const float inv = 1.0f / det;
+                            const float t = T * inv, u = V * inv, v = W * inv;
+                            if (t > tmin && t < tmax) {
+                                uint off2 = toff; asm volatile("" : "+v"(off2));
+                                const f32x4 rx = *reinterpret_cast<const f32x4*>(trisBase + off2), ry = *reinterpret_cast<const f32x4*>(trisBase + (off2 + 16u)), rz = *reinterpret_cast<const f32x4*>(trisBase + (off2 + 32u));
+                                const uint prim = __float_as_uint(rx.w), flags = __float_as_uint(ry.w);
+                                bool c = ((t < bestT) || (t == bestT && prim < bestPrim)) && ((t < lt) || (t == lt && prim < lp));
+                                if (c) c = t8_tri_box_accepts(rx, ry, rz, rz.w, o.x, o.y, o.z, ix, iy, iz, t);
+                                if (c && (flags & 1u)) c = alpha_test_slot(sc, slot0 + h + T8_LANES * r, u, v);
+                                if (c) { lt = t; lp = prim; lu = u; lv = v; }
+                            }
+                        }
+                    }
+                }
+                const bool cand = (lp != 0xFFFFFFFFu);
+                if (t8_ballot(cand) != 0ull) {
+                    if (cand) { minePrim = lp; mineUV[threadIdx.x] = make_float2(lu, lv); }
+                    float tk = lt; uint pkk = lp;
+                    {   float ot = dpp_f<DPP_QP_XOR1>(tk); uint op = dpp_u<DPP_QP_XOR1>(pkk);
+                        bool take = (ot < tk) || (ot == tk && op < pkk); tk = take ? ot : tk; pkk = take ? op : pkk; }
+                    if (pkk != 0xFFFFFFFFu) { bestT = tk; bestPrim = pkk; }
+                    uint m = valid ? __float_as_uint(bestT) : 0u;
+                    m = t8k_max(m, dpp_u<DPP_QP_XOR2>(m)); m = t8k_max(m, dpp_u<DPP_ROW_ROR(4)>(m)); m = t8k_max(m, dpp_u<DPP_ROW_ROR(8)>(m));
+                    maxBest = t8k_max(t8k_max((uint)__builtin_amdgcn_readlane((int)m, 0), (uint)__builtin_amdgcn_readlane((int)m, 16)),
+                                      t8k_max((uint)__builtin_amdgcn_readlane((int)m, 32), (uint)__builtin_amdgcn_readlane((int)m, 48)));
+                }
+                cur = BVH_EMPTY;
+            }
+        }
+
+        if (handOff) {
+            const uint n = (count - i0 < T8_PACKET_RAYS) ? count - i0 : T8_PACKET_RAYS;
+            uint base = 0u;
+            if (lane == 0u) base = atomicAdd(pk.leftoverCount, n);
+            base = t8k_uniform(base);
+            if (base + n <= pk.capacity) { if (valid && h == 0u) pk.leftover[base + (lane >> 1)] = i; }
+            else if (lane == 0u) atomicOr(overflowFlag, 2u);
+        } else if (valid) {
+            if (bestPrim == 0xFFFFFFFFu) { if (h == 0u) { HitInfo hh; hh.t = bestT; hh.prim = 0xFFFFFFFFu; hh.u = hh.v = 0.f; commit(i, hh); } }
+            else if (minePrim == bestPrim) { const float2 uv = mineUV[threadIdx.x]; HitInfo hh; hh.t = bestT; hh.prim = bestPrim; hh.u = uv.x; hh.v = uv.y; commit(i, hh); }
+        }
+    }
+}
+
+}
diff --git a/rtxpt_amd/csrc/pt_wavefront.h b/rtxpt_amd/csrc/pt_wavefront.h
--- a/rtxpt_amd/csrc/pt_wavefront.h
+++ b/rtxpt_amd/csrc/pt_wavefront.h
@@ -22,12 +22,20 @@
     FirstVertexCamera firstCamera;
 };
 
-static const uint TRAV_COUNTERS = 5, TRAV_RESOLVE = 4, PASS_COUNTERS = 16, PASS_SHADOW_OFFSET = 5, PASS_CLASS_OFFSET = 10;
+static const uint TRAV_COUNTERS = 5, TRAV_RESOLVE = 4, PASS_COUNTERS = 16, PASS_SHADOW_OFFSET = 5, PASS_CLASS_OFFSET = 10, PASS_LEFTOVER = 14;
 struct TravAux { TravTask* taskQ[2]; uint* counts; uint taskCap; unsigned long long* bestKey; uint* resolveList; const uint* primToSlot; uint maxBlocks; };
 
 void launch_generate(const PathKernelContext& k, PathPool pool, const uint* ownedPixels, uint numOwned, uint sampleFirst, uint spp, uint first, uint n, uint* queue, uint* countPtr, hipStream_t st);
 void launch_extend(const DeviceScene& sc, PathPool pool, const uint* queue, const uint* countPtr, uint count, WaveCounters* wc, bool counters, TravAux aux, hipStream_t st, bool ranged = false);
-void launch_extend_first(const PathKernelContext& k, PathPool pool, FirstVertex fv, const uint* countPtr, uint count, WaveCounters* wc, TravAux aux, hipStream_t st);
+#ifndef T8_PACKET_STACK
+#define T8_PACKET_STACK 64
+#endif
+#ifndef T8_PACKET_STEP_CAP
+#define T8_PACKET_STEP_CAP 128
+#endif
+static const uint T8_PACKET_RAYS = 32;
+struct FirstPackets { uint* leftover; uint* leftoverCount; uint capacity, stepCap, stackBound; };
+void launch_extend_first(const PathKernelContext& k, PathPool pool, FirstVertex fv, const uint* countPtr, uint count, WaveCounters* wc, TravAux aux, FirstPackets pk, hipStream_t st);
 void launch_shade(const PathKernelContext& k, PathPool pool, const uint* queueIn, const uint* countInPtr, uint countIn, uint* queueOut, uint* countOutPtr,
                   ShadowQueue sq, WaveCounters* wc, uint* classScratch, uint* classCount, hipStream_t st, PathPool outPool = PathPool{},
                   const FirstVertex* fv = nullptr, const uint* inertBits = nullptr);
diff --git a/rtxpt_amd/csrc/pt_wavefront.hip b/rtxpt_amd/csrc/pt_wavefront.hip
--- a/rtxpt_amd/csrc/pt_wavefront.hip
+++ b/rtxpt_amd/csrc/pt_wavefront.hip
@@ -1,6 +1,7 @@
 #include "pt_wavefront.h"
 #include "pt_traverse8.h"
 #include "pt_traverse8p.h"
+#include "pt_traverse8k.h"
 #include "pt_wavefront_device.h"
 #include <cstdlib>
 #define T8_TRAVERSE traverse8_pairs
@@ -28,15 +29,17 @@
     if (countPtr && t == 0u) atomicAdd(countPtr, n);
 }
 
-template <bool COUNT, bool RANGED, bool FIRST = false>
+template <bool COUNT, bool RANGED, bool FIRST = false, bool LISTED = false>
 __device__ __forceinline__ void t8_extend_body(const DeviceScene& sc, const PathPool& pool, const uint* __restrict__ queue, const uint count, WaveCounters* wc, const TravAux& aux, const uint rpc,
                                                uint2* stack, uint* rayBuf, float2* mineUV, const uint vBlock, const uint vGrid, const FirstVertex* fv = nullptr) {
     static_assert(!FIRST || (!COUNT && !RANGED), "vertex 0 in place: composed frames only");
+    static_assert(!LISTED || FIRST, "an index list: vertex 0 in place only");
     Traverse8Counters ctr; t8_counters_init(ctr);
     auto fetch = [&](uint i, float3& o, float3& d, float& tmin, float& tmax, uint& startRef, float& bestT0, uint& bestPrim0) -> uint {
         if (FIRST) {
             asm volatile("" ::: "memory");
             const FirstVertexCamera fc = wc->firstCamera;
+            if (LISTED) i = queue[i];
             uint px, sample; first_vertex_of(*fv, i, px, sample);
             PathKernelContext::cameraRay(fc.cam, fc.perPixelJitterAAScale, px >> 16, px & 0xFFFFu, sample, o, d);
             tmin = 0.0f; tmax = kMaxRayTravel; startRef = 0u; bestT0 = kMaxRayTravel; bestPrim0 = 0xFFFFFFFFu;
@@ -70,6 +73,26 @@
     __shared__ uint rayBuf[T8_RAYBUF_WORDS];
     __shared__ float2 mineUV[T8_BLOCK];
     t8_extend_body<false, false, true>(sc, pool, nullptr, *countPtr, wc, aux, rpc, stack, rayBuf, mineUV, blockIdx.x, gridDim.x, &fv);
+}
+
+__global__ void __launch_bounds__(T8_BLOCK, T8_EXTEND_MIN_BLOCKS) k_extend_first_packets(DeviceScene sc, PathPool pool, FirstVertex fv, const uint* __restrict__ countPtr, WaveCounters* wc, FirstPackets pk) {
+    __shared__ uint2 stack[(T8_BLOCK / 64u) * T8_PACKET_STACK];
+    __shared__ float2 mineUV[T8_BLOCK];
+    auto form = [&](uint i, float3& o, float3& d) {
+        asm volatile("" ::: "memory");
+        const FirstVertexCamera fc = wc->firstCamera;
+        uint px, sample; first_vertex_of(fv, i, px, sample);
+        PathKernelContext::cameraRay(fc.cam, fc.perPixelJitterAAScale, px >> 16, px & 0xFFFFu, sample, o, d);
+    };
+    auto commit = [&](uint p, const HitInfo& h) { pool.hit[p] = make_uint4(asuint(h.t), h.prim, asuint(h.u), asuint(h.v)); };
+    traverse8_packets(sc, *countPtr, stack, mineUV, form, commit, pk, &wc->overflow);
+}
+__global__ void __launch_bounds__(T8_BLOCK, T8_EXTEND_MIN_BLOCKS) k_extend_first_listed(DeviceScene sc, PathPool pool, FirstVertex fv, FirstPackets pk, WaveCounters* wc, TravAux aux, uint rpc) {
+    __shared__ uint2 stack[T8_GROUPS_PER_BLOCK * BVH8_STACK_STRIDE];
+    __shared__ uint rayBuf[T8_RAYBUF_WORDS];
+    __shared__ float2 mineUV[T8_BLOCK];
+    uint n = *pk.leftoverCount; if (n > pk.capacity) n = pk.capacity;
+    t8_extend_body<false, false, true, true>(sc, pool, pk.leftover, n, wc, aux, rpc, stack, rayBuf, mineUV, blockIdx.x, gridDim.x, &fv);
 }
 
 __global__ void __launch_bounds__(256) k_first_split_rays(PathKernelContext k, PathPool pool, FirstVertex fv, TravAux aux) {
@@ -732,9 +755,14 @@
 static const uint T8_SWEEP_BLOCKS = 2048;
 static inline uint shadow_resolve_grid(uint count) { const uint g = grid_for(count, 256u, T8_SWEEP_BLOCKS); return g < T8_RESOLVE_BLOCKS ? T8_RESOLVE_BLOCKS : g; }
 static void launch_extend_stragglers(const DeviceScene& sc, PathPool pool, uint count, WaveCounters* wc, TravAux aux, hipStream_t st);
-void launch_extend_first(const PathKernelContext& k, PathPool pool, FirstVertex fv, const uint* countPtr, uint count, WaveCounters* wc, TravAux aux, hipStream_t st) {
+void launch_extend_first(const PathKernelContext& k, PathPool pool, FirstVertex fv, const uint* countPtr, uint count, WaveCounters* wc, TravAux aux, FirstPackets pk, hipStream_t st) {
     const uint rpc = rays_per_chunk(count);
     const uint g = grid_for(count, (T8_BLOCK / 64u) * rpc * T8_CHUNKS_PER_WAVE_MIN, (aux.maxBlocks && aux.maxBlocks < T8_MAX_BLOCKS) ? aux.maxBlocks : T8_MAX_BLOCKS);
+    if (pk.leftover) {
+        const uint gp = grid_for(count, (T8_BLOCK / 64u) * T8_PACKET_RAYS, (aux.maxBlocks && aux.maxBlocks < T8_MAX_BLOCKS) ? aux.maxBlocks : T8_MAX_BLOCKS);
+        hipLaunchKernelGGL(k_extend_first_packets, dim3(gp), dim3(T8_BLOCK), 0, st, k.sc, pool, fv, countPtr, wc, pk);
+        hipLaunchKernelGGL(k_extend_first_listed, dim3(g), dim3(T8_BLOCK), 0, st, k.sc, pool, fv, pk, wc, aux, rpc);
+    } else
     hipLaunchKernelGGL(k_extend_first, dim3(g), dim3(T8_BLOCK), 0, st, k.sc, pool, fv, countPtr, wc, aux, rpc);
     hipLaunchKernelGGL(k_first_split_rays, dim3(T8_RESOLVE_BLOCKS), dim3(256), 0, st, k, pool, fv, aux);
     launch_extend_stragglers(k.sc, pool, count, wc, aux, st);
```

Result: faster. 1997 Mrays/s (median of 6 runs) (+4.4%).
